# angeris/cfmm-routing-code

Hardware: NVIDIA H100
Metric: pools x dual-evaluations / second (1M constant-product pools, 4096 tokens); time to 1e-6 rel-gap reported beside it (higher is better)
Workload: dtype f64

## Files before the change

### cfmm_routing_code_b200/_lib.py

```python
from __future__ import annotations

import ctypes as C
import os

from . import build as _build

KIND_PRODUCT, KIND_SUM, KIND_GEOMEAN, KIND_BOUNDED = 0, 1, 2, 3

_ERRORS = {
    -1: "CFMM_E_NULL (required pointer is NULL)",
    -2: "CFMM_E_KIND (unknown kind / unsupported arity)",
    -3: "CFMM_E_SIZE (bad size)",
    -4: "CFMM_E_CUDA (CUDA runtime error)",
    -5: "CFMM_E_NODEVICE (no sm_90 device)",
    -6: "CFMM_E_STATE (handle used in the wrong state)",
}


class CfmmError(RuntimeError):
    pass


class Bucket(C.Structure):
    _fields_ = [
        ("kind", C.c_int32), ("arity", C.c_int32), ("n_pools", C.c_int64), ("stride", C.c_int64),
        ("reserves", C.c_void_p), ("tok_idx", C.c_void_p), ("gamma", C.c_void_p),
        ("weights", C.c_void_p), ("logrw", C.c_void_p), ("theta_bar", C.c_void_p),
    ]


class BlockedPairs(C.Structure):
    _fields_ = [
        ("n_pools", C.c_int64), ("n_tiles", C.c_int64), ("pools_per_tile", C.c_int32), ("reserved", C.c_int32),
        ("r0", C.c_void_p), ("r1", C.c_void_p), ("gamma_inv", C.c_void_p), ("lid", C.c_void_p),
        ("pos", C.c_void_p), ("rows", C.c_void_p), ("tok", C.c_void_p), ("desc", C.c_void_p),
    ]


class SolveParams(C.Structure):
    _fields_ = [("tol", C.c_double), ("nu_floor", C.c_double), ("max_iter", C.c_int32), ("cg_max", C.c_int32)]


class SolveResult(C.Structure):
    _fields_ = [("dual_value", C.c_double), ("primal_value", C.c_double), ("gap", C.c_double),
                ("primal_infeas", C.c_double), ("err", C.c_double), ("iters", C.c_int32), ("evals", C.c_int32),
                ("hvps", C.c_int32), ("status", C.c_int32)]


class PeerCtx(C.Structure):
    _fields_ = [("recv_acc_dev", C.c_void_p), ("recv_vec_dev", C.c_void_p), ("rank", C.c_int32), ("world", C.c_int32),
                ("seq_acc", C.c_uint64), ("seq_vec", C.c_uint64)]


class CsrPools(C.Structure):
    _fields_ = [("n_tokens", C.c_int32), ("n_pools", C.c_int64), ("nnz", C.c_int64), ("pool_ptr", C.c_void_p),
                ("tok_idx", C.c_void_p), ("reserves", C.c_void_p), ("weights", C.c_void_p), ("logrw", C.c_void_p),
                ("gamma", C.c_void_p), ("kind", C.c_void_p)]


class Batch(C.Structure):
    _fields_ = [("n_problems", C.c_int32), ("pool_range", C.c_void_p), ("c", C.c_void_p), ("a", C.c_void_p),
                ("flags", C.c_void_p), ("nu", C.c_void_p), ("psi", C.c_void_p), ("stats", C.c_void_p),
                ("delta", C.c_void_p), ("lambda_", C.c_void_p), ("trade_stride", C.c_int64)]


class BatchParams(C.Structure):
    _fields_ = [("tol", C.c_double), ("eps0", C.c_double), ("eps_min", C.c_double), ("eps_shrink", C.c_double),
                ("floor_rel", C.c_double), ("max_outer", C.c_int32), ("max_inner", C.c_int32)]


class EvalOut(C.Structure):
    _fields_ = [("delta", C.c_void_p), ("lambda_", C.c_void_p), ("hcoef", C.c_void_p), ("hmask", C.c_void_p)]


_lib = None


def lib_path() -> str:
    return _build.LIB


def load(build_if_missing: bool = True):
    global _lib
    if _lib is not None:
        return _lib
    path = _build.LIB
    if build_if_missing and _build.needs_build():
        try:
            _build.build_library()
        except Exception as e:
            if not os.path.exists(path):
                raise CfmmError(f"libcfmm_b200.so is missing and could not be built: {e}") from e
    if not os.path.exists(path):
        raise CfmmError("libcfmm_b200.so is missing: run `python -c 'import __graft_entry__ as g; g.build()'`")
    lib = C.CDLL(path)
    vp, i32, i64, dbl = C.c_void_p, C.c_int32, C.c_int64, C.c_double
    lib.cfmm_arb_eval.argtypes = [C.POINTER(Bucket), i32, vp, vp, dbl, vp, vp, C.POINTER(EvalOut), vp]
    lib.cfmm_arb_eval.restype = C.c_int
    for name in ("cfmm_hvp", "cfmm_hess_diag", "cfmm_hess_dense"):
        fn = getattr(lib, name)
        fn.restype = C.c_int
    lib.cfmm_hvp.argtypes = [C.POINTER(Bucket), i32, vp, vp, vp, vp, vp]
    lib.cfmm_hess_diag.argtypes = [C.POINTER(Bucket), i32, vp, vp, vp, vp]
    lib.cfmm_hess_dense.argtypes = [C.POINTER(Bucket), i32, vp, vp, vp, vp]
    lib.cfmm_blocked_layout_info.argtypes = [C.POINTER(i32)] * 4
    lib.cfmm_blocked_layout_info.restype = C.c_int
    lib.cfmm_set_blocked_config.argtypes = [i32]
    lib.cfmm_set_blocked_config.restype = C.c_int
    lib.cfmm_blocked_build_work_bytes.argtypes = [i64]
    lib.cfmm_blocked_build_work_bytes.restype = i64
    lib.cfmm_blocked_build.argtypes = [i64, i32, vp, vp, vp, C.POINTER(BlockedPairs), vp, vp, vp, i64, vp]
    lib.cfmm_blocked_build.restype = C.c_int
    lib.cfmm_blocked_eval.argtypes = [C.POINTER(BlockedPairs), i32, vp, vp, vp, C.POINTER(EvalOut), vp, i64, vp]
    lib.cfmm_blocked_eval.restype = C.c_int
    lib.cfmm_blocked_hvp.argtypes = [C.POINTER(BlockedPairs), i32, vp, vp, vp, vp, vp]
    lib.cfmm_blocked_hvp.restype = C.c_int
    lib.cfmm_blocked_diag.argtypes = [C.POINTER(BlockedPairs), i32, vp, vp, vp]
    lib.cfmm_blocked_diag.restype = C.c_int
    lib.cfmm_blocked_dense.argtypes = [C.POINTER(BlockedPairs), i32, vp, vp, vp]
    lib.cfmm_blocked_dense.restype = C.c_int
    lib.cfmm_blocked_solve_work_bytes.argtypes = [C.POINTER(BlockedPairs), i32]
    lib.cfmm_blocked_solve_work_bytes.restype = i64
    lib.cfmm_blocked_solve.argtypes = [C.POINTER(BlockedPairs), i32, vp, vp, vp, vp, vp, vp, vp,
                                       C.POINTER(SolveParams), C.POINTER(SolveResult), vp]
    lib.cfmm_blocked_solve.restype = C.c_int
    lib.cfmm_blocked_solve_peer.argtypes = [C.POINTER(BlockedPairs), i32, vp, vp, vp, vp, vp, vp, vp,
                                            C.POINTER(SolveParams), C.POINTER(SolveResult), C.POINTER(PeerCtx), vp]
    lib.cfmm_blocked_solve_peer.restype = C.c_int
    lib.cfmm_persist_solve_work_bytes.argtypes = [C.POINTER(BlockedPairs), i32]
    lib.cfmm_persist_solve_work_bytes.restype = i64
    lib.cfmm_persist_solve.argtypes = lib.cfmm_blocked_solve_peer.argtypes
    lib.cfmm_persist_solve.restype = C.c_int
    lib.cfmm_set_persist_cooperative.argtypes = [i32]
    lib.cfmm_set_persist_cooperative.restype = C.c_int
    lib.cfmm_persist_last_profile.argtypes = [vp]
    lib.cfmm_persist_last_profile.restype = C.c_int
    lib.cfmm_batch_solve_work_bytes.argtypes = [C.POINTER(CsrPools), i32, i64]
    lib.cfmm_batch_solve_work_bytes.restype = i64
    lib.cfmm_set_batch_lanes.argtypes = [i32]
    lib.cfmm_set_batch_lanes.restype = C.c_int
    lib.cfmm_batch_solve.argtypes = [C.POINTER(CsrPools), C.POINTER(Batch), C.POINTER(BatchParams), vp, vp]
    lib.cfmm_batch_solve.restype = C.c_int
    lib.cfmm_allreduce_ll.argtypes = [vp, vp, i32, i32, i32, i64, i64, vp, C.c_uint64, vp]
    lib.cfmm_allreduce_ll.restype = C.c_int
    lib.cfmm_sum_update_multipliers.argtypes = [C.POINTER(Bucket), vp, vp, vp, vp]
    lib.cfmm_sum_update_multipliers.restype = C.c_int
    lib.cfmm_zero.argtypes = [vp, i64, vp]
    lib.cfmm_zero.restype = C.c_int
    lib.cfmm_set_scatter_mode.argtypes = [i32]
    lib.cfmm_set_scatter_mode.restype = C.c_int
    lib.cfmm_launch_count.restype = i64
    lib.cfmm_reset_launch_count.restype = None
    lib.cfmm_last_cuda_error.restype = C.c_char_p
    lib.cfmm_version.restype = C.c_char_p
    if os.environ.get("CFMM_BATCH_LANES"):
        lib.cfmm_set_batch_lanes(int(os.environ["CFMM_BATCH_LANES"]))
    if os.environ.get("CFMM_BLOCKED_CFG"):
        for c in os.environ["CFMM_BLOCKED_CFG"].split(","):
            lib.cfmm_set_blocked_config(int(c))
    _lib = lib
    return lib


def check(rc: int, what: str = "cfmm call"):
    if rc != 0:
        extra = ""
        if rc == -4 and _lib is not None:
            extra = ": " + _lib.cfmm_last_cuda_error().decode()
        raise CfmmError(f"{what} failed: {_ERRORS.get(rc, rc)}{extra}")
```

### cfmm_routing_code_b200/csrc/cfmm_blocked.cu

```cuda
#include <math.h>

#include "cfmm_blocked.cuh"

using namespace cfmm;

namespace {

template <int P, int THREADS, int STAGES, int MODE , bool TRADES, bool HESS>
__global__ void __launch_bounds__(THREADS, kCtasPerSm)
k_blocked(const BlockedArgs A) {
    extern __shared__ __align__(128) unsigned char smem_raw[];
    __shared__ uint64_t full[STAGES];
    __shared__ double part[THREADS / 32];
    if (threadIdx.x == 0) {
        for (int s = 0; s < STAGES; ++s) mbar_init(&full[s], 1);
        mbar_fence_init();
    }
    __syncthreads();
    const long long t_beg = (A.n_tiles * (long long)blockIdx.x) / gridDim.x;
    const long long t_end = (A.n_tiles * (long long)(blockIdx.x + 1)) / gridDim.x;
    double acc = 0.0, acc2 = 0.0;
    unsigned phase = 0;
    blocked_pass<P, THREADS, STAGES, MODE, TRADES, HESS, false, true>(A, smem_raw, full, phase, t_beg, t_end, acc, acc2);
    if (MODE == 0) cta_accumulate<THREADS>(acc, part, A.arb);
}

template <int P>
struct __align__(128) TabStage {
    uint32_t rows[BlockedCfg<P>::kRowsMax];
    int32_t tok[BlockedCfg<P>::kTokMax];
    int4 desc;
};

template <int P>
__device__ __forceinline__ void issue_tables(TabStage<P>* st, uint64_t* bar, const BlockedArgs& A, long long tile,
                                             const int4 d) {
    const unsigned rows_b = round16(4u * (unsigned)d.y);
    const unsigned tok_b = round16(4u * (unsigned)d.x);
    mbar_expect_tx(bar, 16u + rows_b + tok_b);
    bulk_g2s(&st->desc, A.desc + tile, 16, bar);
    bulk_g2s(st->rows, A.rows + tile * BlockedCfg<P>::kRowsMax, rows_b, bar);
    bulk_g2s(st->tok, A.tok + tile * BlockedCfg<P>::kTokMax, tok_b, bar);
}

template <int NF>
struct PoolRegs {
    double a[NF];
    uint32_t lid, pos;
};

template <int P, int THREADS, int NF, int NPOOL>
__device__ __forceinline__ void load_pools(PoolRegs<NF> (&r)[NPOOL], const BlockedArgs& A, long long tile, int tid) {
    const long long toff = tile * P;
#pragma unroll
    for (int u = 0; u < NPOOL; ++u) {
        const long long q = toff + tid + u * THREADS;
#pragma unroll
        for (int k = 0; k < NF; ++k) r[u].a[k] = __ldg(A.slab[k] + q);
        r[u].lid = __ldg(A.lid + q);
        r[u].pos = __ldg(A.pos + q);
    }
}

template <int P, int NF>
__device__ __forceinline__ void prefetch_pools_l2(const BlockedArgs& A, long long tile) {
    constexpr int tp = P;
    const long long toff = tile * P;
#pragma unroll
    for (int k = 0; k < NF; ++k) bulk_prefetch_l2(A.slab[k] + toff, tp * 8);
    bulk_prefetch_l2(A.lid + toff, tp * 4);
    bulk_prefetch_l2(A.pos + toff, tp * 4);
}

template <int P, int THREADS, int STAGES, int MODE, bool TRADES, bool HESS>
__global__ void __launch_bounds__(THREADS, kCtasPerSm)
k_blocked_regs(const BlockedArgs A) {
    constexpr int NF = (MODE == 0) ? 3 : 1;
    constexpr int NPOOL = P / THREADS;
    constexpr int NPRE = (P + THREADS - 1) / THREADS;
    using St = TabStage<P>;
    extern __shared__ __align__(128) unsigned char smem_raw[];
    St* stages = reinterpret_cast<St*>(smem_raw);
    double* nul0 = reinterpret_cast<double*>(smem_raw + (size_t)STAGES * sizeof(St));
    double* g0 = nul0 + 2 * P;
    __shared__ uint64_t full[STAGES];
    __shared__ double part[THREADS / 32];
    const int tid = threadIdx.x, lane = tid & 31, warp = tid >> 5;
    const long long t_beg = (A.n_tiles * (long long)blockIdx.x) / gridDim.x;
    const long long t_end = (A.n_tiles * (long long)(blockIdx.x + 1)) / gridDim.x;
    if (tid == 0) {
        for (int s = 0; s < STAGES; ++s) mbar_init(&full[s], 1);
        mbar_fence_init();
    }
    __syncthreads();
    if (tid == 0) {
        for (int s = 0; s < STAGES; ++s) {
            const long long t = t_beg + s;
            if (t < t_end) issue_tables<P>(&stages[s], &full[s], A, t, __ldg(A.desc + t));
        }
        if (t_beg + 1 < t_end) prefetch_pools_l2<P, NF>(A, t_beg + 1);
        if (t_beg + 2 < t_end) prefetch_pools_l2<P, NF>(A, t_beg + 2);
    }
    PoolRegs<NF> cur[NPOOL], nxt[NPOOL];
    if (t_beg < t_end) load_pools<P, THREADS, NF, NPOOL>(cur, A, t_beg, tid);
    asm volatile("griddepcontrol.wait;" ::: "memory");
    asm volatile("griddepcontrol.launch_dependents;" ::: "memory");
    for (int j = blockIdx.x * THREADS + tid; j < A.n_zero; j += gridDim.x * THREADS) A.zero_next[j] = 0.0;
    double acc = 0.0;
    if (t_beg < t_end) {
        mbar_wait(&full[0], 0);
        if (MODE != 2) {
            const int ntok = stages[0].desc.x;
            for (int t = tid; t < ntok; t += THREADS) nul0[t] = __ldg(A.vec + stages[0].tok[t]);
        }
    }
    __syncthreads();
    int stage = 0, pstage = 0, buf = 0;
    unsigned parity = 0;
    for (long long tile = t_beg; tile < t_end; ++tile) {
        St& S = stages[stage];
        const double* nul = nul0 + buf * P;
        double* g = g0 + buf * 2 * P;
        const long long nx = tile + 1;
        int nstage = stage + 1;
        unsigned nparity = parity;
        if (nstage == STAGES) { nstage = 0; nparity ^= 1u; }
        double pre[NPRE];
        int ntok_n = 0;
        if (tid == 0 && tile + 3 < t_end) prefetch_pools_l2<P, NF>(A, tile + 3);
        if (nx < t_end) {
            load_pools<P, THREADS, NF, NPOOL>(nxt, A, nx, tid);
            mbar_wait(&full[nstage], nparity);
            if (MODE != 2) {
                ntok_n = stages[nstage].desc.x;
#pragma unroll
                for (int k = 0; k < NPRE; ++k) {
                    const int t = tid + k * THREADS;
                    pre[k] = (t < ntok_n) ? __ldg(A.vec + stages[nstage].tok[t]) : 0.0;
                }
            }
        }
        {
            double f0[NPOOL], f1[NPOOL];
#pragma unroll
            for (int u = 0; u < NPOOL; ++u) {
                const uint32_t li = cur[u].lid;
                if (MODE == 0) {
                    EvalOp::apply<TRADES, HESS>(A, tile * P + tid + u * THREADS, cur[u].a[0], cur[u].a[NF > 1 ? 1 : 0],
                                                cur[u].a[NF > 2 ? 2 : 0], nul[li & 0xffffu], nul[li >> 16], f0[u], f1[u],
                                                acc);
                } else if (MODE == 1) {
                    f0[u] = cur[u].a[0] * (nul[li & 0xffffu] - nul[li >> 16]);
                    f1[u] = -f0[u];
                } else {
                    f0[u] = cur[u].a[0];
                    f1[u] = f0[u];
                }
            }
#pragma unroll
            for (int u = 0; u < NPOOL; ++u) {
                g[cur[u].pos & 0xffffu] = f0[u];
                g[cur[u].pos >> 16] = f1[u];
            }
        }
        if (MODE != 2 && nx < t_end) {
            double* nn = nul0 + (buf ^ 1) * P;
#pragma unroll
            for (int k = 0; k < NPRE; ++k) {
                const int t = tid + k * THREADS;
                if (t < ntok_n) nn[t] = pre[k];
            }
        }
        __syncthreads();
        if (tid == 0 && tile > t_beg) {
            const long long far = tile - 1 + STAGES;
            if (far < t_end) {
                fence_proxy_async();
                issue_tables<P>(&stages[pstage], &full[pstage], A, far, __ldg(A.desc + far));
            }
        }
        const int nrow = S.desc.y;
        for (int r = tid; r < nrow; r += THREADS) {
            const uint32_t rw = S.rows[r];
            const double* q = g + row_start(rw);
            const int len = row_len(rw);
            double s0 = 0.0, s1 = 0.0;
            int k = 0;
#pragma unroll 1
            for (; k + 4 <= len; k += 4) { s0 += q[k] + q[k + 2]; s1 += q[k + 1] + q[k + 3]; }
            if (k + 2 <= len) { s0 += q[k]; s1 += q[k + 1]; k += 2; }
            if (k < len) s0 += q[k];
            const double s = s0 + s1;
            if (s != 0.0) atomicAdd(A.out + S.tok[row_tok(rw)], s);
        }
#pragma unroll
        for (int u = 0; u < NPOOL; ++u) cur[u] = nxt[u];
        pstage = stage; stage = nstage; parity = nparity; buf ^= 1;
    }
    if (MODE == 0) {
        acc = warp_sum(acc);
        if (lane == 0) part[warp] = acc;
        __syncthreads();
        if (tid < 32) {
            double s = (tid < THREADS / 32) ? part[tid] : 0.0;
            s = warp_sum(s);
            if (tid == 0 && s != 0.0) atomicAdd(A.arb, s);
        }
    }
}

__global__ void __launch_bounds__(256)
k_blocked_dense(long long n_pools, int n, const uint32_t* __restrict__ lid, const int32_t* __restrict__ tok,
                const double* __restrict__ hcoef, double* H) {
    for (long long q = (long long)blockIdx.x * blockDim.x + threadIdx.x; q < n_pools; q += (long long)gridDim.x * blockDim.x) {
        const double h = hcoef[q];
        if (h != 0.0) {
            const long long tile = q / kTileP;
            const uint32_t li = lid[q];
            const long long a = tok[tile * BlockedCfg<kTileP>::kTokMax + (li & 0xffffu)];
            const long long b = tok[tile * BlockedCfg<kTileP>::kTokMax + (li >> 16)];
            atomicAdd(H + a * n + a, h); atomicAdd(H + b * n + b, h);
            atomicAdd(H + a * n + b, -h); atomicAdd(H + b * n + a, -h);
        }
    }
}

int g_pdl = 1;
int g_row_cap = 32;

template <int MODE, bool TRADES, bool HESS>
int launch_tma(const BlockedArgs& A, cudaStream_t st) {
    constexpr int NF = (MODE == 0) ? 3 : 1;
    auto kern = k_blocked<kTileP, kTileT, kTileStages, MODE, TRADES, HESS>;
    const size_t sm = pass_smem_bytes<kTileP, kTileStages>(NF);
    static bool attr = false;
    if (!attr) {
        cudaFuncSetAttribute(kern, cudaFuncAttributeMaxDynamicSharedMemorySize, (int)sm);
        attr = true;
    }
    const long long cap = (long long)kCtasPerSm * num_sms();
    const int grid = (int)(A.n_tiles < cap ? A.n_tiles : cap);
    cudaLaunchConfig_t cfg = {};
    cfg.gridDim = dim3(grid); cfg.blockDim = dim3(kTileT); cfg.dynamicSmemBytes = sm; cfg.stream = st;
    cudaLaunchAttribute at[1];
    at[0].id = cudaLaunchAttributeProgrammaticStreamSerialization;
    at[0].val.programmaticStreamSerializationAllowed = g_pdl;
    cfg.attrs = at; cfg.numAttrs = 1;
    cudaLaunchKernelEx(&cfg, kern, A);
    return check_launch();
}

template <int MODE>
int launch_regs(const BlockedArgs& A, cudaStream_t st) {
    constexpr int P = kTileP, T = kTileT, S = 4;
    auto kern = k_blocked_regs<P, T, S, MODE, false, false>;
    const size_t sm = (size_t)S * sizeof(TabStage<P>) + (size_t)(2 * P + 4 * P) * sizeof(double);
    static bool attr = false;
    if (!attr) {
        cudaFuncSetAttribute(kern, cudaFuncAttributeMaxDynamicSharedMemorySize, (int)sm);
        attr = true;
    }
    const long long cap = (long long)kCtasPerSm * num_sms();
    const int grid = (int)(A.n_tiles < cap ? A.n_tiles : cap);
    cudaLaunchConfig_t cfg = {};
    cfg.gridDim = dim3(grid); cfg.blockDim = dim3(T); cfg.dynamicSmemBytes = sm; cfg.stream = st;
    cudaLaunchAttribute at[1];
    at[0].id = cudaLaunchAttributeProgrammaticStreamSerialization;
    at[0].val.programmaticStreamSerializationAllowed = g_pdl;
    cfg.attrs = at; cfg.numAttrs = 1;
    cudaLaunchKernelEx(&cfg, kern, A);
    return check_launch();
}

}

namespace cfmm {

int fill_blocked_args(const cfmm_blocked_pairs* b, BlockedArgs& A) {
    if (!b) return CFMM_E_NULL;
    if (b->pools_per_tile != kTileP) return CFMM_E_KIND;
    if (b->n_tiles < 0 || b->n_pools < 0 || b->n_pools > b->n_tiles * (int64_t)kTileP) return CFMM_E_SIZE;
    if (b->n_tiles > 0 && (!b->lid || !b->pos || !b->rows || !b->tok || !b->desc)) return CFMM_E_NULL;
    A.n_tiles = b->n_tiles;
    A.M = b->n_tiles * (int64_t)kTileP;
    A.lid = b->lid; A.pos = b->pos; A.rows = b->rows; A.tok = b->tok;
    A.desc = reinterpret_cast<const int4*>(b->desc);
    A.zero_next = nullptr; A.n_zero = 0;
    A.slab[0] = A.slab[1] = A.slab[2] = nullptr;
    A.vec = nullptr; A.vec2 = nullptr; A.beta = 0.0;
    A.out = nullptr; A.arb = nullptr; A.delta = A.lambda = A.hcoef = nullptr;
    return CFMM_OK;
}

}

extern "C" {

int cfmm_blocked_layout_info(int32_t* pools_per_tile, int32_t* rows_stride, int32_t* tok_stride, int32_t* row_cap) {
    if (pools_per_tile) *pools_per_tile = kTileP;
    if (rows_stride) *rows_stride = BlockedCfg<kTileP>::kRowsMax;
    if (tok_stride) *tok_stride = BlockedCfg<kTileP>::kTokMax;
    if (row_cap) *row_cap = g_row_cap;
    return CFMM_OK;
}

int cfmm_set_blocked_config(int32_t cfg) {
    if (cfg >= 300) { const int c = cfg - 300; if (c < 8 || c > 32) return CFMM_E_KIND; g_row_cap = c; return CFMM_OK; }
    if (cfg == 200 || cfg == 201) { g_pdl = cfg - 200; return CFMM_OK; }
    return CFMM_E_KIND;
}

int cfmm_blocked_eval(const cfmm_blocked_pairs* b, int32_t n_tokens, const double* nu, double* psi, double* arb,
                      const cfmm_eval_out* out, double* zero_next, int64_t n_zero, void* stream) {
    BlockedArgs A;
    int rc = fill_blocked_args(b, A);
    if (rc) return rc;
    if (n_tokens <= 0) return CFMM_E_SIZE;
    if (!nu || !psi || !arb) return CFMM_E_NULL;
    if (b->n_tiles == 0) return CFMM_OK;
    if (!b->r0 || !b->r1 || !b->gamma_inv) return CFMM_E_NULL;
    A.slab[0] = b->r0; A.slab[1] = b->r1; A.slab[2] = b->gamma_inv;
    A.vec = nu; A.out = psi; A.arb = arb;
    A.zero_next = zero_next; A.n_zero = zero_next ? (int)n_zero : 0;
    const bool trades = out && out->delta && out->lambda;
    const bool hess = out && out->hcoef;
    if (trades) { A.delta = out->delta; A.lambda = out->lambda; }
    if (hess) A.hcoef = out->hcoef;
    cudaStream_t st = static_cast<cudaStream_t>(stream);
    if (trades && hess) return launch_tma<0, true, true>(A, st);
    if (trades) return launch_tma<0, true, false>(A, st);
    if (hess) return launch_tma<0, false, true>(A, st);
    return launch_tma<0, false, false>(A, st);
}

int cfmm_blocked_hvp(const cfmm_blocked_pairs* b, int32_t n_tokens, const double* hcoef, const double* vt, double* y,
                     double* zero_next, void* stream) {
    BlockedArgs A;
    int rc = fill_blocked_args(b, A);
    if (rc) return rc;
    if (n_tokens <= 0) return CFMM_E_SIZE;
    if (!hcoef || !vt || !y) return CFMM_E_NULL;
    if (b->n_tiles == 0) return CFMM_OK;
    A.slab[0] = hcoef; A.vec = vt; A.out = y;
    A.zero_next = zero_next; A.n_zero = zero_next ? n_tokens : 0;
    return launch_regs<1>(A, static_cast<cudaStream_t>(stream));
}

int cfmm_blocked_dense(const cfmm_blocked_pairs* b, int32_t n_tokens, const double* hcoef, double* H, void* stream) {
    BlockedArgs A;
    int rc = fill_blocked_args(b, A);
    if (rc) return rc;
    if (n_tokens <= 0) return CFMM_E_SIZE;
    if (!hcoef || !H) return CFMM_E_NULL;
    if (b->n_tiles == 0) return CFMM_OK;
    const long long total = b->n_tiles * (long long)kTileP;
    const long long need = (total + 255) / 256, cap = 8LL * num_sms();
    k_blocked_dense<<<(int)(need < cap ? need : cap), 256, 0, static_cast<cudaStream_t>(stream)>>>(total, n_tokens, b->lid, b->tok, hcoef, H);
    return check_launch();
}

int cfmm_blocked_diag(const cfmm_blocked_pairs* b, int32_t n_tokens, const double* hcoef, double* diag, void* stream) {
    BlockedArgs A;
    int rc = fill_blocked_args(b, A);
    if (rc) return rc;
    if (n_tokens <= 0) return CFMM_E_SIZE;
    if (!hcoef || !diag) return CFMM_E_NULL;
    if (b->n_tiles == 0) return CFMM_OK;
    A.slab[0] = hcoef; A.out = diag;
    return launch_regs<2>(A, static_cast<cudaStream_t>(stream));
}

}
```

### cfmm_routing_code_b200/csrc/cfmm_blocked.cuh

```cuda
#pragma once
#include <math.h>

#include "cfmm_dev.cuh"

namespace cfmm {

#ifndef CFMM_TILE_P
#define CFMM_TILE_P 1024
#endif
#ifndef CFMM_CTAS_PER_SM
#define CFMM_CTAS_PER_SM 2
#endif
constexpr int kTileP = CFMM_TILE_P;
constexpr int kTileT = kTileP / 2;
constexpr int kTileStages = 2;
constexpr int kCtasPerSm = CFMM_CTAS_PER_SM;
static_assert(kTileP % 64 == 0 && kTileP <= 1024, "tile size: whole warps of two-pool threads, 10-bit local token ids");

template <int P>
struct BlockedCfg {
    static constexpr int kTokMax = P;
    static constexpr int kRowCapMin = 8;
    static constexpr int kRowsMax = P + 2 * P / kRowCapMin + 8;
};

template <int P, int NF>
struct __align__(128) Stage {
    double a[NF][P];
    uint32_t lid[P];
    uint32_t pos[P];
    uint32_t rows[BlockedCfg<P>::kRowsMax];
    int32_t tok[BlockedCfg<P>::kTokMax];
    int4 desc;
};

struct BlockedArgs {
    long long n_tiles;
    long long M;
    const double* slab[3];
    const uint32_t* lid;
    const uint32_t* pos;
    const uint32_t* rows;
    const int32_t* tok;
    const int4* desc;
    const double* vec;
    const double* vec2;
    double beta;
    double* out;
    double* zero_next;
    int n_zero;
    double* arb;
    double* delta;
    double* lambda;
    double* hcoef;
};

__device__ __forceinline__ unsigned round16(unsigned bytes) { return (bytes + 15u) & ~15u; }

template <int P, int NF>
__device__ __forceinline__ void issue_tile(Stage<P, NF>* st, uint64_t* bar, const BlockedArgs& A, long long tile,
                                           const int4 d) {
    const unsigned rows_b = round16(4u * (unsigned)d.y);
    const unsigned tok_b = round16(4u * (unsigned)d.x);
    const long long off = tile * P;
    mbar_expect_tx(bar, (unsigned)(NF * P * 8 + P * 4 + P * 4 + 16) + rows_b + tok_b);
    bulk_g2s(&st->desc, A.desc + tile, 16, bar);
#pragma unroll
    for (int k = 0; k < NF; ++k) bulk_g2s(st->a[k], A.slab[k] + off, P * 8, bar);
    bulk_g2s(st->lid, A.lid + off, P * 4, bar);
    bulk_g2s(st->pos, A.pos + off, P * 4, bar);
    bulk_g2s(st->rows, A.rows + tile * BlockedCfg<P>::kRowsMax, rows_b, bar);
    bulk_g2s(st->tok, A.tok + tile * BlockedCfg<P>::kTokMax, tok_b, bar);
}

__device__ __forceinline__ double clamp0(double x) {
    const int hi = __double2hiint(x);
    const int m = ~(hi >> 31);
    return __hiloint2double(hi & m, __double2loint(x) & m);
}

struct EvalOp {
    template <bool TRADES, bool HESS>
    __device__ __forceinline__ static void apply(const BlockedArgs& A, long long q, double R0, double R1, double gi,
                                                 double n0, double n1, double& f0, double& f1, double& acc) {
        const double p0 = n0 * R0, p1 = n1 * R1;
        const double w = p0 * p1 * gi;
        const double v = rsqrt(w);
        const double a = p0 * v, b = p1 * v;
        const double ob = 1.0 - b, oa = 1.0 - a;
        const double r0 = fma(-b, gi, 1.0), r1 = fma(-a, gi, 1.0);
        const double x0 = (ob < 0.0) ? ob * gi : clamp0(r0);
        const double x1 = (oa < 0.0) ? oa * gi : clamp0(r1);
        f0 = R0 * x0;
        f1 = R1 * x1;
        acc = fma(n0, f0, fma(n1, f1, acc));
        if (TRADES) {
            A.delta[q] = f0 < 0.0 ? -f0 : 0.0; A.delta[A.M + q] = f1 < 0.0 ? -f1 : 0.0;
            A.lambda[q] = f0 > 0.0 ? f0 : 0.0; A.lambda[A.M + q] = f1 > 0.0 ? f1 : 0.0;
        }
        if (HESS) A.hcoef[q] = (x0 != 0.0 || x1 != 0.0) ? 0.5 * w * v : 0.0;
    }
};

__device__ __forceinline__ int row_start(uint32_t r) { return (int)(r & 0xffffu); }
__device__ __forceinline__ int row_len(uint32_t r) { return (int)((r >> 16) & 0x3fu); }
__device__ __forceinline__ int row_tok(uint32_t r) { return (int)(r >> 22); }

template <bool COHERENT>
__device__ __forceinline__ double load_vec(const double* p) { return COHERENT ? *p : __ldg(p); }
template <int MODE, bool COHERENT>
__device__ __forceinline__ double gather_vec(const BlockedArgs& A, int t) {
    if (MODE == 1 && COHERENT) return fma(A.beta, A.vec[t], A.vec2[t]);
    return load_vec<COHERENT>(A.vec + t);
}

template <int P, int STAGES>
constexpr size_t pass_smem_bytes(int nf) {
    return (size_t)STAGES * (nf == 3 ? sizeof(Stage<P, 3>) : sizeof(Stage<P, 1>)) + (size_t)(3 * P) * sizeof(double);
}

template <int P, int THREADS, int STAGES, int MODE, bool TRADES, bool HESS, bool COHERENT, bool PDL>
__device__ __forceinline__ void blocked_pass(const BlockedArgs& A, unsigned char* smem_raw, uint64_t* full, unsigned& phase,
                                             long long t_beg, long long t_end, double& acc, double& acc2) {
    constexpr int NF = (MODE == 0) ? 3 : 1;
    using St = Stage<P, NF>;
    St* stages = reinterpret_cast<St*>(smem_raw);
    double* nul = reinterpret_cast<double*>(smem_raw + (size_t)STAGES * sizeof(St));
    double* g = nul + P;
    const int tid = threadIdx.x;
    if (tid == 0) {
        for (int s = 0; s < STAGES; ++s) {
            const long long t = t_beg + s;
            if (t < t_end) issue_tile<P, NF>(&stages[s], &full[s], A, t, __ldg(A.desc + t));
        }
    }
    if (PDL) {
        asm volatile("griddepcontrol.wait;" ::: "memory");
        asm volatile("griddepcontrol.launch_dependents;" ::: "memory");
    }
    for (int j = blockIdx.x * THREADS + tid; j < A.n_zero; j += gridDim.x * THREADS) A.zero_next[j] = 0.0;
    int stage = 0;
    constexpr int NPRE = (P + THREADS - 1) / THREADS;
    if (t_beg < t_end) {
        mbar_wait(&full[0], phase & 1u);
        if (MODE != 2) {
            const int ntok = stages[0].desc.x;
            for (int t = tid; t < ntok; t += THREADS) nul[t] = gather_vec<MODE, COHERENT>(A, stages[0].tok[t]);
        }
    }
    __syncthreads();
    for (long long tile = t_beg; tile < t_end; ++tile) {
        St& S = stages[stage];
        phase ^= 1u << stage;
        const int4 d = S.desc;
        const long long far = tile + STAGES;
        int4 dfar = make_int4(0, 0, 0, 0);
        if (tid == 0 && far < t_end) dfar = __ldg(A.desc + far);
        {
            constexpr int NPOOL = P / THREADS;
            double f0[NPOOL], f1[NPOOL];
            uint32_t ps[NPOOL];
#pragma unroll
            for (int u = 0; u < NPOOL; ++u) {
                const int l = tid + u * THREADS;
                const uint32_t li = S.lid[l];
                ps[u] = S.pos[l];
                if (MODE == 0) {
                    EvalOp::apply<TRADES, HESS>(A, tile * P + l, S.a[0][l], S.a[NF > 1 ? 1 : 0][l], S.a[NF > 2 ? 2 : 0][l],
                                                nul[li & 0xffffu], nul[li >> 16], f0[u], f1[u], acc);
                } else if (MODE == 1) {
                    const double pa = nul[li & 0xffffu], pb = nul[li >> 16], h = S.a[0][l];
                    f0[u] = h * (pa - pb);
                    f1[u] = -f0[u];
                    if (COHERENT) {
                        acc = fma(f0[u], pa - pb, acc);
                        acc2 = fma(h, fma(pa, pa, pb * pb), acc2);
                    }
                } else {
                    f0[u] = S.a[0][l];
                    f1[u] = f0[u];
                }
            }
#pragma unroll
            for (int u = 0; u < NPOOL; ++u) {
                g[ps[u] & 0xffffu] = f0[u];
                g[ps[u] >> 16] = f1[u];
            }
        }
        __syncthreads();
        const long long nxt = tile + 1;
        const int nstage = (stage + 1 == STAGES) ? 0 : stage + 1;
        double pre[NPRE];
        int ntok_n = 0;
        if (nxt < t_end) {
            mbar_wait(&full[nstage], (phase >> nstage) & 1u);
            if (MODE != 2) {
                ntok_n = stages[nstage].desc.x;
#pragma unroll
                for (int k = 0; k < NPRE; ++k) {
                    const int t = tid + k * THREADS;
                    pre[k] = (t < ntok_n) ? gather_vec<MODE, COHERENT>(A, stages[nstage].tok[t]) : 0.0;
                }
            }
        }
        for (int r = tid; r < d.y; r += THREADS) {
            const uint32_t rw = S.rows[r];
            const double* q = g + row_start(rw);
            const int len = row_len(rw);
            double s0 = 0.0, s1 = 0.0;
            int k = 0;
#pragma unroll 1
            for (; k + 4 <= len; k += 4) { s0 += q[k] + q[k + 2]; s1 += q[k + 1] + q[k + 3]; }
            if (k + 2 <= len) { s0 += q[k]; s1 += q[k + 1]; k += 2; }
            if (k < len) s0 += q[k];
            const double s = s0 + s1;
            if (s != 0.0) atomicAdd(A.out + S.tok[row_tok(rw)], s);
        }
        if (MODE != 2 && nxt < t_end) {
#pragma unroll
            for (int k = 0; k < NPRE; ++k) {
                const int t = tid + k * THREADS;
                if (t < ntok_n) nul[t] = pre[k];
            }
        }
        __syncthreads();
        if (tid == 0 && far < t_end) {
            fence_proxy_async();
            issue_tile<P, NF>(&S, &full[stage], A, far, dfar);
        }
        stage = nstage;
    }
}

template <int THREADS>
__device__ __forceinline__ void cta_accumulate(double acc, double* part, double* target) {
    const int tid = threadIdx.x;
    acc = warp_sum(acc);
    if ((tid & 31) == 0) part[tid >> 5] = acc;
    __syncthreads();
    if (tid < 32) {
        double s = (tid < THREADS / 32) ? part[tid] : 0.0;
        s = warp_sum(s);
        if (tid == 0 && s != 0.0) atomicAdd(target, s);
    }
}

int fill_blocked_args(const cfmm_blocked_pairs* b, BlockedArgs& A);

}
```

### cfmm_routing_code_b200/csrc/cfmm_layout.cu

```cuda
#include <cub/cub.cuh>

#include "cfmm_blocked.cuh"

using namespace cfmm;

namespace {

constexpr int LT = kTileT;
constexpr int LP = kTileP;
constexpr int LH = 2 * kTileP;
constexpr int LI = 4;
static_assert(LT * LI == LH, "block sort shape");
constexpr int LR = BlockedCfg<kTileP>::kRowsMax;

struct BuildArgs {
    long long m;
    int n_tokens, nb, row_cap, key_bits, tok_bits;
    const int32_t* idx;
    const double* R;
    const double* gamma;
    const uint32_t* order;
    double *r0, *r1, *gi;
    uint32_t *lid, *pos;
    uint32_t* rows;
    int32_t* tok;
    int4* desc;
    int32_t* status;
};

__global__ void __launch_bounds__(256)
k_pool_keys(long long m, int n_tokens, int nb, const int32_t* __restrict__ idx, const double* __restrict__ R,
            const double* __restrict__ gamma, uint32_t* __restrict__ keys, uint32_t* __restrict__ vals, int32_t* status) {
    int bad = 0;
    for (long long i = (long long)blockIdx.x * blockDim.x + threadIdx.x; i < m; i += (long long)gridDim.x * blockDim.x) {
        const int a = idx[2 * i], b = idx[2 * i + 1];
        const double R0 = R[2 * i], R1 = R[2 * i + 1], g = gamma[i];
        const bool ok = a >= 0 && a < n_tokens && b >= 0 && b < n_tokens && a != b && R0 > 0.0 && R1 > 0.0 && isfinite(R0) &&
                        isfinite(R1) && g > 0.0 && g <= 1.0;
        bad |= ok ? 0 : 1;
        const long long ba = ok ? ((long long)a * nb) / n_tokens : 0, bb = ok ? ((long long)b * nb) / n_tokens : 0;
        keys[i] = (uint32_t)((ba * nb + bb) * n_tokens + (ok ? a : 0));
        vals[i] = (uint32_t)i;
    }
    if (__syncthreads_or(bad) && threadIdx.x == 0) atomicAdd(status + 1, 1);
}

using Sort = cub::BlockRadixSort<uint32_t, LT, LI, uint32_t>;
using Scan = cub::BlockScan<int, LT>;

struct TileSmem {
    union { typename Sort::TempStorage sort; typename Scan::TempStorage scan; } tmp;
    uint32_t sk[LH];
    uint32_t sv[LH];
    uint16_t gid[LH];
    int gs[LP + 2];
    int rfirst[LP + 1];
    uint16_t rrank[LR + 8];
    int rstart[LR + 8];
    uint16_t lidh[LP][2], posh[LP][2];
    int ntok, nrow;
};

__global__ void __launch_bounds__(LT)
k_build_tiles(const BuildArgs B) {
    extern __shared__ __align__(16) unsigned char tile_smem_raw[];
    TileSmem& M = *reinterpret_cast<TileSmem*>(tile_smem_raw);
    auto& tmp = M.tmp;
    uint32_t* sk = M.sk; uint32_t* sv = M.sv; uint16_t* gid = M.gid; int* gs = M.gs; int* rfirst = M.rfirst;
    uint32_t* rk = M.sk;
    uint16_t* rrank = M.rrank; int* rstart = M.rstart;
    auto& lidh = M.lidh; auto& posh = M.posh;
    int& s_ntok = M.ntok; int& s_nrow = M.nrow;
    const int tid = threadIdx.x;
    const long long tile = blockIdx.x;
    const long long p0 = tile * LP;
    const int np = (int)(B.m - p0 < LP ? B.m - p0 : LP);
    const int nh = 2 * np;
    uint32_t key[LI], val[LI];
#pragma unroll
    for (int u = 0; u < LI; ++u) {
        const int h = tid * LI + u;
        const int slot = h >= LP ? 1 : 0, l = h - slot * LP;
        if (l < np) {
            const uint32_t pool = B.order[p0 + l];
            key[u] = (uint32_t)B.idx[2 * (long long)pool + slot];
            val[u] = (uint32_t)(slot << 15 | l);
        } else {
            key[u] = 0xffffffffu; val[u] = 0u;
        }
    }
    Sort(tmp.sort).Sort(key, val, 0, 32);
#pragma unroll
    for (int u = 0; u < LI; ++u) { sk[tid * LI + u] = key[u]; sv[tid * LI + u] = val[u]; }
    __syncthreads();
    int head[LI], gpre[LI];
#pragma unroll
    for (int u = 0; u < LI; ++u) {
        const int i = tid * LI + u;
        head[u] = (i < nh && (i == 0 || sk[i] != sk[i - 1])) ? 1 : 0;
    }
    int ntok;
    Scan(tmp.scan).ExclusiveSum(head, gpre, ntok);
    __syncthreads();
    const bool bad = ntok > LP;
#pragma unroll
    for (int u = 0; u < LI; ++u) {
        const int i = tid * LI + u;
        if (i < nh) {
            const int g = gpre[u] + head[u] - 1;
            gid[i] = (uint16_t)g;
            if (head[u] && !bad) { gs[g] = i; B.tok[tile * LP + g] = (int32_t)sk[i]; }
        }
    }
    if (tid == 0) { s_ntok = ntok; if (!bad) gs[ntok] = nh; }
    __syncthreads();
    if (bad) {
        if (tid == 0) { atomicAdd(B.status, 1); B.desc[tile] = make_int4(0, 0, 0, 0); }
        for (int l = tid; l < LP; l += LT) {
            B.r0[p0 + l] = 1.0; B.r1[p0 + l] = 1.0; B.gi[p0 + l] = 1.0; B.lid[p0 + l] = 0u; B.pos[p0 + l] = 0u;
        }
        return;
    }
    const int cap = B.row_cap;
    int nsub[2], rpre[2];
#pragma unroll
    for (int u = 0; u < 2; ++u) {
        const int g = tid * 2 + u;
        nsub[u] = g < ntok ? (gs[g + 1] - gs[g] + cap - 1) / cap : 0;
    }
    int nrow;
    Scan(tmp.scan).ExclusiveSum(nsub, rpre, nrow);
    __syncthreads();
#pragma unroll
    for (int u = 0; u < 2; ++u) {
        const int g = tid * 2 + u;
        if (g < ntok) {
            rfirst[g] = rpre[u];
            const int cnt = gs[g + 1] - gs[g];
            for (int s = 0; s < nsub[u]; ++s) {
                const int len = min(cap, cnt - cap * s);
                rk[rpre[u] + s] = (uint32_t)(63 - len) << 16 | (uint32_t)(rpre[u] + s);
            }
        }
    }
    if (tid == 0) s_nrow = nrow;
    __syncthreads();
    uint32_t rkey[LI], rdum[LI];
#pragma unroll
    for (int u = 0; u < LI; ++u) {
        const int r = tid * LI + u;
        rkey[u] = r < nrow ? rk[r] : 0xffffffffu;
        rdum[u] = 0u;
    }
    __syncthreads();
    Sort(tmp.sort).Sort(rkey, rdum, 0, 22);
    int rlen[LI], spre[LI];
#pragma unroll
    for (int u = 0; u < LI; ++u) {
        const int r = tid * LI + u;
        rlen[u] = r < nrow ? 63 - (int)(rkey[u] >> 16) : 0;
        if (r < nrow) rrank[rkey[u] & 0xffffu] = (uint16_t)r;
    }
    __syncthreads();
    int total;
    Scan(tmp.scan).ExclusiveSum(rlen, spre, total);
#pragma unroll
    for (int u = 0; u < LI; ++u) {
        const int r = tid * LI + u;
        if (r < nrow) { rstart[r] = spre[u]; rk[r] = (uint32_t)rlen[u]; }
    }
    __syncthreads();
    for (int i = tid; i < nh; i += LT) {
        const int g = gid[i], o = i - gs[g];
        const int r = rrank[rfirst[g] + o / cap];
        const int p = rstart[r] + o % cap;
        const uint32_t v = sv[i];
        const int slot = v >> 15, l = v & 0x7fffu;
        lidh[l][slot] = (uint16_t)g;
        posh[l][slot] = (uint16_t)p;
        if (o % cap == 0) B.rows[tile * LR + r] = (uint32_t)rstart[r] | rk[r] << 16 | (uint32_t)g << 22;
    }
    __syncthreads();
    for (int l = tid; l < LP; l += LT) {
        if (l < np) {
            const uint32_t pool = B.order[p0 + l];
            B.lid[p0 + l] = (uint32_t)lidh[l][0] | (uint32_t)lidh[l][1] << 16;
            B.pos[p0 + l] = (uint32_t)posh[l][0] | (uint32_t)posh[l][1] << 16;
            B.r0[p0 + l] = B.R[2 * (long long)pool]; B.r1[p0 + l] = B.R[2 * (long long)pool + 1];
            B.gi[p0 + l] = 1.0 / B.gamma[pool];
        } else {
            const int pl = l - np;
            B.lid[p0 + l] = 0u;
            B.pos[p0 + l] = (uint32_t)(nh + 2 * pl) | (uint32_t)(nh + 2 * pl + 1) << 16;
            B.r0[p0 + l] = 1.0; B.r1[p0 + l] = 1.0; B.gi[p0 + l] = 1.0;
        }
    }
    if (tid == 0) { B.desc[tile] = make_int4(s_ntok, s_nrow, 0, 0); atomicAdd(B.status + 2, s_nrow); }
}

inline size_t align_up(size_t x) { return (x + 255) & ~(size_t)255; }

size_t sort_temp_bytes(long long m) {
    size_t bytes = 0;
    cub::DeviceRadixSort::SortPairs(nullptr, bytes, (const uint32_t*)nullptr, (uint32_t*)nullptr, (const uint32_t*)nullptr,
                                    (uint32_t*)nullptr, (int)m, 0, 32);
    return bytes;
}

}

extern "C" {

int64_t cfmm_blocked_build_work_bytes(int64_t n_pools) {
    if (n_pools <= 0 || n_pools > 0x7fffffffLL) return CFMM_E_SIZE;
    return (int64_t)(4 * align_up(4 * (size_t)n_pools) + align_up(sort_temp_bytes(n_pools)));
}

int cfmm_blocked_build(int64_t n_pools, int32_t n_tokens, const int32_t* idx, const double* reserves, const double* gamma,
                       const cfmm_blocked_pairs* out, uint32_t* order, int32_t* status, void* work, int64_t work_bytes,
                       void* stream) {
    if (!idx || !reserves || !gamma || !out || !order || !status || !work) return CFMM_E_NULL;
    if (n_pools <= 0 || n_pools > 0x7fffffffLL || n_tokens <= 0) return CFMM_E_SIZE;
    if (work_bytes < cfmm_blocked_build_work_bytes(n_pools)) return CFMM_E_SIZE;
    const long long T = (n_pools + LP - 1) / LP;
    if (out->pools_per_tile != LP || out->n_tiles != T || out->n_pools != n_pools) return CFMM_E_SIZE;
    if (!out->r0 || !out->r1 || !out->gamma_inv || !out->lid || !out->pos || !out->rows || !out->tok || !out->desc) return CFMM_E_NULL;
    int row_cap = 32;
    cfmm_blocked_layout_info(nullptr, nullptr, nullptr, &row_cap);
    long long nb = (long long)llround(sqrt((double)n_pools / LP));
    if (nb < 1) nb = 1;
    if ((double)nb * nb * n_tokens >= 4294967296.0) return CFMM_E_SIZE;
    int key_bits = 1;
    while (key_bits < 32 && (1ull << key_bits) < (unsigned long long)(nb * nb) * (unsigned long long)n_tokens) ++key_bits;
    cudaStream_t st = static_cast<cudaStream_t>(stream);
    unsigned char* w = static_cast<unsigned char*>(work);
    auto take = [&](size_t bytes) { unsigned char* p = w; w += align_up(bytes); return p; };
    uint32_t* keys = reinterpret_cast<uint32_t*>(take(4 * (size_t)n_pools));
    uint32_t* vals = reinterpret_cast<uint32_t*>(take(4 * (size_t)n_pools));
    uint32_t* keys2 = reinterpret_cast<uint32_t*>(take(4 * (size_t)n_pools));
    take(4 * (size_t)n_pools);
    size_t temp_bytes = sort_temp_bytes(n_pools);
    void* temp = take(temp_bytes);
    cudaMemsetAsync(status, 0, 16, st);
    const int grid = (int)((n_pools + 255) / 256 < 4LL * num_sms() ? (n_pools + 255) / 256 : 4LL * num_sms());
    k_pool_keys<<<grid, 256, 0, st>>>(n_pools, n_tokens, (int)nb, idx, reserves, gamma, keys, vals, status);
    int rc = check_launch();
    if (rc) return rc;
    if (cub::DeviceRadixSort::SortPairs(temp, temp_bytes, keys, keys2, vals, order, (int)n_pools, 0, key_bits, st) != cudaSuccess) {
        g_last_err = cudaGetLastError();
        return CFMM_E_CUDA;
    }
    BuildArgs B;
    B.m = n_pools; B.n_tokens = n_tokens; B.nb = (int)nb; B.row_cap = row_cap; B.key_bits = key_bits; B.tok_bits = 32;
    B.idx = idx; B.R = reserves; B.gamma = gamma; B.order = order;
    B.r0 = const_cast<double*>(out->r0); B.r1 = const_cast<double*>(out->r1); B.gi = const_cast<double*>(out->gamma_inv);
    B.lid = const_cast<uint32_t*>(out->lid); B.pos = const_cast<uint32_t*>(out->pos);
    B.rows = const_cast<uint32_t*>(out->rows); B.tok = const_cast<int32_t*>(out->tok);
    B.desc = reinterpret_cast<int4*>(const_cast<int32_t*>(out->desc));
    B.status = status;
    static bool attr = false;
    if (!attr) {
        cudaFuncSetAttribute(k_build_tiles, cudaFuncAttributeMaxDynamicSharedMemorySize, (int)sizeof(TileSmem));
        attr = true;
    }
    k_build_tiles<<<(int)T, LT, sizeof(TileSmem), st>>>(B);
    return check_launch();
}

}
```

### cfmm_routing_code_b200/csrc/cfmm_persist.cu

```cuda
#include <math.h>
#include <string.h>

#include "cfmm_blocked.cuh"

using namespace cfmm;

namespace {

constexpr int PT = kTileT;
constexpr unsigned long long kSpinLimit = 6000000000ull;


struct DevResult {
    double dual_value, primal_value, gap, primal_infeas, err;
    int iters, evals, hvps, status;
    unsigned long long seq_acc, seq_vec;
    long long prof[16];
};

struct PersistArgs {
    BlockedArgs B;
    int n;
    const double *c, *a;
    const unsigned char *eq, *fixed;
    double* nu[2];
    double* acc[2];
    double *y, *diag, *hcoef;
    double *lb, *grad[2], *fr[2], *pg[2], *dt, *x, *r, *z, *p, *minv;
    unsigned* ctl;
    double tol, nu_floor;
    int max_iter, cg_max;
    LLCell* const* recv_acc;
    LLCell* const* recv_vec;
    int rank, world;
    unsigned long long seq_acc, seq_vec;
    double* nu_out;
    double* psi_out;
    DevResult* res;
};

__device__ __forceinline__ unsigned ld_acquire_gpu(const unsigned* p) {
    unsigned v;
    asm volatile("ld.acquire.gpu.global.u32 %0, [%1];" : "=r"(v) : "l"(p) : "memory");
    return v;
}

struct Kkt { double err, g, primal, infeas, lin; };

template <int MODE>
__device__ __forceinline__ void run_pass(const PersistArgs& S, const double* vec, double* out, unsigned char* smem_raw,
                                         uint64_t* full, unsigned& phase, long long t_beg, long long t_end, double* part,
                                         double beta) {
    BlockedArgs A = S.B;
    A.vec = vec; A.out = out; A.zero_next = nullptr; A.n_zero = 0;
    asm volatile("fence.proxy.async;" ::: "memory");
    if (MODE == 0) { A.arb = out + S.n; A.hcoef = S.hcoef; }
    else A.slab[0] = S.hcoef;
    if (MODE == 1) { A.vec2 = S.z; A.beta = beta; }
    double acc = 0.0, acc2 = 0.0;
    blocked_pass<kTileP, PT, kTileStages, MODE, false, MODE == 0, true, false>(A, smem_raw, full, phase, t_beg, t_end, acc, acc2);
    if (MODE == 0) {
        cta_accumulate<PT>(acc, part, A.arb);
        asm volatile("fence.proxy.async;" ::: "memory");
    }
    if (MODE == 1) {
        cta_accumulate<PT>(acc, part, out + S.n);
        __syncthreads();
        cta_accumulate<PT>(acc2, part, out + S.n + 1);
    }
}

__device__ __forceinline__ double ldw(const double* p) { return *p; }

constexpr int kSliceMax = 256;
constexpr int kQ = 10;

enum { PH_KKT = 1, PH_DIAG = 2, PH_HVP = 3, PH_STEP = 4, PH_DONE = 5 };

struct DistArgs {
    PersistArgs P;
    double* accr[2];
    double* y2[2];
    double* partial;
    int nsl;
};

struct DState {
    int phase, set, cur, iters, evals, hvps, status, cg_k, ls, yb, first_step, dir_ok, aborted, parity;
    double err, g0, rz, r0n, eta, alpha, lin1, beta, al, imx, thr;
    int flat;
    Kkt kc;
    unsigned long long seq_acc, seq_vec;
    unsigned bar;
    long long prof[16];
};

__device__ __forceinline__ void grid_barrier(unsigned* ctl, DState* ds) {
    __threadfence();
    __syncthreads();
    if (threadIdx.x == 0) {
        const unsigned target = (++ds->bar) * gridDim.x;
        atomicAdd(ctl, 1u);
        const long long t0 = clock64();
        while (ld_acquire_gpu(ctl) < target) {
            if (ld_acquire_gpu(ctl + 32) != 0u) { ds->aborted = 1; break; }
            if ((unsigned long long)(clock64() - t0) > kSpinLimit) { ctl[32] = 1u; ds->aborted = 1; break; }
        }
    }
    __syncthreads();
}

__device__ __forceinline__ void ll_push(double mine, LLCell* const* recv, long long slot, long long stride, int j, int rank,
                                        int world, unsigned long long seq) {
    for (int r = 0; r < world; ++r)
        if (r != rank) st_ll(recv[r] + slot + (long long)rank * stride + j, mine, seq);
}
__device__ __noinline__ double ll_poll_sum(double mine, LLCell* const* recv, long long slot, long long stride, int j,
                                           int rank, int world, unsigned long long seq, unsigned* ctl) {
    const LLCell* base = recv[rank] + slot + j;
    const long long t0 = clock64();
    double s = 0.0;
    for (int r0 = 0; r0 < world; r0 += 4) {
        double v0 = 0.0, v1 = 0.0, v2 = 0.0, v3 = 0.0;
        unsigned pending = 0u;
#pragma unroll
        for (int k = 0; k < 4; ++k)
            if (r0 + k < world && r0 + k != rank) pending |= 1u << k;
        unsigned spins = 0u;
        while (pending) {
            double t[4];
            unsigned long long f[4];
#pragma unroll
            for (int k = 0; k < 4; ++k)
                if (pending >> k & 1u) ld_ll(base + (long long)(r0 + k) * stride, t[k], f[k]);
            if ((pending & 1u) && f[0] == seq) { v0 = t[0]; pending &= ~1u; }
            if ((pending & 2u) && f[1] == seq) { v1 = t[1]; pending &= ~2u; }
            if ((pending & 4u) && f[2] == seq) { v2 = t[2]; pending &= ~4u; }
            if ((pending & 8u) && f[3] == seq) { v3 = t[3]; pending &= ~8u; }
            if (pending && (++spins & 63u) == 0u && (unsigned long long)(clock64() - t0) > kSpinLimit) { ctl[32] = 1u; break; }
        }
        if (r0 + 0 < world) s += (r0 + 0 == rank) ? mine : v0;
        if (r0 + 1 < world) s += (r0 + 1 == rank) ? mine : v1;
        if (r0 + 2 < world) s += (r0 + 2 == rank) ? mine : v2;
        if (r0 + 3 < world) s += (r0 + 3 == rank) ? mine : v3;
    }
    return s;
}

template <bool MULTI>
__global__ void __launch_bounds__(PT, kCtasPerSm)
k_solve_dist(const __grid_constant__ DistArgs D) {
    extern __shared__ __align__(128) unsigned char smem_raw[];
    __shared__ uint64_t full[kTileStages];
    __shared__ double part[PT / 32];
    __shared__ double tot[kQ];
    __shared__ DState ds;
    const PersistArgs& S = D.P;
    const int tid = threadIdx.x, lane = tid & 31, warp = tid >> 5;
    const int n = S.n, nsl = D.nsl, G = gridDim.x;
    if (tid == 0) {
        for (int s = 0; s < kTileStages; ++s) mbar_init(&full[s], 1);
        mbar_fence_init();
        ds.phase = PH_KKT; ds.set = 0; ds.cur = 0; ds.iters = 0; ds.evals = 0; ds.hvps = 0; ds.status = 1; ds.cg_k = 0; ds.ls = 0;
        ds.yb = 0; ds.first_step = 1; ds.dir_ok = 0; ds.aborted = 0; ds.parity = 0; ds.flat = 0;
        ds.err = INFINITY; ds.g0 = 0.0; ds.rz = 0.0; ds.r0n = 0.0; ds.eta = 0.1; ds.alpha = 1.0; ds.lin1 = 0.0; ds.beta = 0.0;
        ds.al = 0.0; ds.imx = 0.0; ds.thr = 1e-5;
        ds.kc.err = INFINITY; ds.kc.g = 0.0; ds.kc.primal = 0.0; ds.kc.infeas = 0.0; ds.kc.lin = 0.0;
        ds.seq_acc = S.seq_acc; ds.seq_vec = S.seq_vec; ds.bar = 0;
        for (int k = 0; k < 16; ++k) ds.prof[k] = 0;
    }
    __syncthreads();
    const long long t_beg = (S.B.n_tiles * (long long)blockIdx.x) / G;
    const long long t_end = (S.B.n_tiles * (long long)(blockIdx.x + 1)) / G;
    unsigned phase_bits = 0;
    for (int s0 = blockIdx.x + warp * G; s0 < nsl; s0 += (PT / 32) * G) {
        const int lo = (int)((long long)n * s0 / nsl), hi = (int)((long long)n * (s0 + 1) / nsl);
        for (int j = lo + lane; j < hi; j += 32) {
            const double l = S.eq[j] ? S.nu_floor : fmax(S.c[j], S.nu_floor);
            S.lb[j] = l;
            S.nu[0][j] = S.fixed[j] ? S.c[j] : fmax(S.nu[0][j], l);
            S.acc[0][j] = 0.0;
        }
        if (s0 == nsl - 1 && lane == 0) S.acc[0][n] = 0.0;
    }
    grid_barrier(S.ctl, &ds);
    for (;;) {
        const int phase = ds.phase, set = ds.set, cur = ds.cur;
        if (phase == PH_DONE || ds.aborted) break;
        const long long tp0 = clock64();
        if (phase == PH_KKT) run_pass<0>(S, S.nu[set], S.acc[set], smem_raw, full, phase_bits, t_beg, t_end, part, 0.0);
        else if (phase == PH_HVP) run_pass<1>(S, S.p, D.y2[ds.yb], smem_raw, full, phase_bits, t_beg, t_end, part, ds.beta);
        else if (phase == PH_DIAG) run_pass<2>(S, nullptr, S.diag, smem_raw, full, phase_bits, t_beg, t_end, part, 0.0);
        const long long tp1 = clock64();
        if (phase != PH_STEP) grid_barrier(S.ctl, &ds);
        const long long tp2 = clock64();
        const int par = ds.parity;
        double* P0 = D.partial + (size_t)par * kQ * kSliceMax;
        constexpr bool multi = MULTI;
        unsigned long long seq = 0;
        if (phase == PH_KKT) seq = ds.seq_acc + 1; else if (phase == PH_DIAG || phase == PH_HVP) seq = ds.seq_vec + 1;
        const long long slot_acc = (long long)(seq % 3) * S.world * (n + 1), slot_vec = (long long)(seq % 3) * S.world * (n + 2);
        if (phase == PH_HVP) {
            const double* yb = D.y2[ds.yb];
            if (multi) {
                for (int s0 = blockIdx.x + warp * G; s0 < nsl; s0 += (PT / 32) * G) {
                    const int lo = (int)((long long)n * s0 / nsl), hi = (int)((long long)n * (s0 + 1) / nsl);
                    for (int j = lo + lane; j < hi; j += 32) ll_push(ldw(yb + j), S.recv_vec, slot_vec, n + 2, j, S.rank, S.world, seq);
                    if (s0 == nsl - 1 && lane < 2) ll_push(ldw(yb + n + lane), S.recv_vec, slot_vec, n + 2, n + lane, S.rank, S.world, seq);
                }
            }
            if (tid == 0) {
                double pHp = ldw(yb + n), pdp = ldw(yb + n + 1);
                if (multi) {
                    pHp = ll_poll_sum(pHp, S.recv_vec, slot_vec, n + 2, n, S.rank, S.world, seq, S.ctl);
                    pdp = ll_poll_sum(pdp, S.recv_vec, slot_vec, n + 2, n + 1, S.rank, S.world, seq, S.ctl);
                }
                ds.flat = pHp <= 1e-14 * pdp;
                ds.al = ds.flat ? 0.0 : ds.rz / pHp;
            }
            __syncthreads();
        }
        const double al = ds.al;
        const int flat = ds.flat;
        for (int s0 = blockIdx.x + warp * G; s0 < nsl; s0 += (PT / 32) * G) {
            const int lo = (int)((long long)n * s0 / nsl), hi = (int)((long long)n * (s0 + 1) / nsl);
            double q[kQ];
#pragma unroll
            for (int k = 0; k < kQ; ++k) q[k] = 0.0;
            for (int j = lo + lane; j < hi; j += 32) {
                if (phase == PH_KKT) {
                    double pj = ldw(S.acc[set] + j);
                    const double nj = ldw(S.nu[set] + j), aj = S.a[j], cj = S.c[j], lbj = ldw(S.lb + j);
                    const unsigned char ej = S.eq[j], fj = S.fixed[j];
                    const bool wl = set != cur;
                    const double np = wl ? ldw(S.nu[cur] + j) : 0.0, gp = wl ? ldw(S.grad[cur] + j) : 0.0;
                    if (multi) {
                        ll_push(pj, S.recv_acc, slot_acc, n + 1, j, S.rank, S.world, seq);
                        if (s0 == nsl - 1 && lane == 0) ll_push(ldw(S.acc[set] + n), S.recv_acc, slot_acc, n + 1, n, S.rank, S.world, seq);
                        pj = ll_poll_sum(pj, S.recv_acc, slot_acc, n + 1, j, S.rank, S.world, seq, S.ctl);
                    }
                    const double g = aj + pj;
                    const bool near = (nj <= lbj * (1.0 + ds.thr)) && !ej;
                    const bool act = fj || (near && g > 0.0);
                    const double f = act ? 0.0 : 1.0, v = nj * g * f;
                    S.grad[set][j] = g; S.fr[set][j] = f; S.pg[set][j] = v; D.accr[set][j] = pj;
                    S.diag[j] = 0.0;
                    q[0] += fabs(v); q[1] += (nj - cj) * aj; q[2] += nj * fabs(g); q[3] += cj * pj;
                    q[4] += nj * (fj ? 0.0 : (ej ? fabs(g) : fmax(-g, 0.0)));
                    q[5] += gp * (nj - np);
                    q[6] = fmax(q[6], fabs(g) * f);
                    q[7] = fmax(q[7], fmax(fabs(aj), fj ? 0.0 : fabs(pj)));
                } else if (phase == PH_DIAG) {
                    double d = ldw(S.diag + j);
                    const double f = ldw(S.fr[cur] + j), g = ldw(S.pg[cur] + j);
                    if (multi) {
                        ll_push(d, S.recv_vec, slot_vec, n + 2, j, S.rank, S.world, seq);
                        d = ll_poll_sum(d, S.recv_vec, slot_vec, n + 2, j, S.rank, S.world, seq, S.ctl);
                    }
                    const double mi = f / fmax(d, 1e-300), r = -g, z = mi * r;
                    S.minv[j] = mi; S.x[j] = 0.0; S.r[j] = r; S.z[j] = z; S.p[j] = z;
                    D.y2[0][j] = 0.0;
                    q[0] += r * z;
                    q[6] = fmax(q[6], fabs(g));
                } else if (phase == PH_HVP) {
                    double yv = ldw(D.y2[ds.yb] + j);
                    const double pp = ldw(S.p + j), zz = ldw(S.z + j), xx = ldw(S.x + j), rr = ldw(S.r + j),
                                 mm = ldw(S.minv + j), g = ldw(S.pg[cur] + j);
                    if (multi) yv = ll_poll_sum(yv, S.recv_vec, slot_vec, n + 2, j, S.rank, S.world, seq, S.ctl);
                    const double pj = fma(ds.beta, pp, zz);
                    double xn = xx;
                    S.p[j] = pj;
                    if (flat) {
                        if (ds.cg_k == 0) { xn = pj; S.x[j] = xn; }
                    } else {
                        const double r = rr - al * yv, z = mm * r;
                        xn = fma(al, pj, xx);
                        S.x[j] = xn; S.r[j] = r; S.z[j] = z;
                        q[0] += r * z;
                    }
                    q[1] += g * xn;
                    D.y2[ds.yb ^ 1][j] = 0.0;
                } else {
                    const double g = ldw(S.pg[cur] + j), xx = ldw(S.x + j), v = ldw(S.nu[cur] + j), l = ldw(S.lb + j);
                    double d;
                    if (ds.first_step) { d = ds.dir_ok ? xx : -g * ds.imx; S.dt[j] = d; }
                    else d = ldw(S.dt + j);
                    const double e = fmin(fmax(ds.alpha * d, -20.0), 20.0);
                    S.nu[cur ^ 1][j] = S.fixed[j] ? S.c[j] : fmax(v * exp(e), l);
                    S.acc[cur ^ 1][j] = 0.0;
                }
            }
            if (s0 == nsl - 1 && lane == 0) {
                if (phase == PH_KKT) {
                    double arb = ldw(S.acc[set] + n);
                    if (multi) arb = ll_poll_sum(arb, S.recv_acc, slot_acc, n + 1, n, S.rank, S.world, seq, S.ctl);
                    q[8] = arb;
                } else if (phase == PH_DIAG) { D.y2[0][n] = 0.0; D.y2[0][n + 1] = 0.0; }
                else if (phase == PH_HVP) { D.y2[ds.yb ^ 1][n] = 0.0; D.y2[ds.yb ^ 1][n + 1] = 0.0; }
                else S.acc[cur ^ 1][n] = 0.0;
            }
            if (phase != PH_STEP) {
#pragma unroll
                for (int k = 0; k < 6; ++k) q[k] = warp_sum(q[k]);
                q[6] = warp_max(q[6]); q[7] = warp_max(q[7]);
                if (lane == 0) {
#pragma unroll
                    for (int k = 0; k < 9; ++k) P0[k * kSliceMax + s0] = q[k];
                }
            }
        }
        const long long tp3 = clock64();
        grid_barrier(S.ctl, &ds);
        const long long tp4 = clock64();
        if (warp < 9 && phase != PH_STEP) {
            const int k = warp;
            const bool is_max = k == 6 || k == 7;
            double t = 0.0;
            for (int s = lane; s < nsl; s += 32) {
                const double v = ldw(P0 + k * kSliceMax + s);
                t = is_max ? fmax(t, v) : t + v;
            }
            t = is_max ? warp_max(t) : warp_sum(t);
            if (lane == 0) tot[k] = t;
        }
        __syncthreads();
        if (tid == 0) {
            ds.parity ^= 1;
            int next = PH_DONE;
            bool newton = false;
            if (ds.aborted) {
                next = PH_DONE;
            } else if (phase == PH_KKT) {
                ++ds.seq_acc; ++ds.evals;
                Kkt k;
                k.g = tot[1] + tot[8];
                k.err = fmax(tot[0] / fmax(fmax(fabs(k.g), 1e-3 * tot[2]), 1e-300), tot[6] / fmax(tot[7], 1e-300));
                k.primal = tot[3]; k.infeas = tot[4] / fmax(fabs(k.g), 1e-300); k.lin = tot[5];
                if (set == cur) {
                    ds.kc = k; ds.err = k.err; ds.g0 = k.g; newton = true;
                } else {
                    if (ds.ls == 0) ds.lin1 = k.lin;
                    bool accept = k.g <= ds.g0 + 1e-4 * k.lin, stalled = false;
                    if (!accept && (fabs(k.g - ds.g0) <= 1e-13 * fabs(ds.g0) || fabs(ds.lin1) <= 1e-9 * fabs(ds.g0))) {
                        if (k.err < 0.99 * ds.err) accept = true;
                        else if (ds.alpha < 1e-3) stalled = true;
                    }
                    if (accept) { ds.cur = set; ds.kc = k; ds.err = k.err; ds.g0 = k.g; newton = true; }
                    else if (stalled || ++ds.ls >= 50) { ds.status = 2; next = PH_DONE; }
                    else { ds.alpha *= 0.5; ds.first_step = 0; next = PH_STEP; }
                }
                if (newton) {
                    if (ds.iters >= S.max_iter) { ds.status = 1; next = PH_DONE; }
                    else {
                        ++ds.iters;
                        if (ds.err <= S.tol) { ds.status = 0; next = PH_DONE; }
                        else next = PH_DIAG;
                    }
                }
            } else if (phase == PH_DIAG) {
                ++ds.seq_vec;
                ds.rz = tot[0]; ds.r0n = sqrt(fmax(ds.rz, 0.0)); ds.eta = fmin(0.1, sqrt(ds.err));
                ds.imx = 1.0 / fmax(tot[6], 1e-300);
                ds.cg_k = 0; ds.beta = 0.0; ds.yb = 0;
                if (ds.rz <= 0.0) { ds.dir_ok = 0; ds.first_step = 1; ds.alpha = 1.0; ds.ls = 0; ds.lin1 = 0.0; next = PH_STEP; }
                else next = PH_HVP;
            } else if (phase == PH_HVP) {
                ++ds.seq_vec; ++ds.hvps;
                bool stop = flat != 0;
                if (!flat) {
                    const double rzn = tot[0];
                    stop = (rzn <= 0.0) || (sqrt(fmax(rzn, 0.0)) <= ds.eta * ds.r0n);
                    ds.beta = rzn / ds.rz;
                    ds.rz = rzn;
                }
                ++ds.cg_k; ds.yb ^= 1;
                if (!stop && ds.cg_k < S.cg_max) next = PH_HVP;
                else {
                    const double sdir = tot[1];
                    ds.dir_ok = (isfinite(sdir) && sdir < 0.0) ? 1 : 0;
                    ds.first_step = 1; ds.alpha = 1.0; ds.ls = 0; ds.lin1 = 0.0;
                    next = PH_STEP;
                }
            } else {
                ds.set = cur ^ 1;
                ds.thr = fmin(1e-2, fmax(1e-3 * (isfinite(ds.err) ? ds.err : 1e-2), 1e-14));
                next = PH_KKT;
            }
            if (next == PH_DONE && ds.status == 1 && ds.err <= S.tol) ds.status = 0;
            ds.phase = next;
            if (blockIdx.x == 0) {
                ds.prof[phase == PH_KKT ? 0 : phase == PH_HVP ? 1 : phase == PH_DIAG ? 2 : 7] += tp1 - tp0;
                ds.prof[3] += tp2 - tp1; ds.prof[4] += tp3 - tp2; ds.prof[5] += tp4 - tp3; ds.prof[6] += clock64() - tp4;
            }
        }
        __syncthreads();
    }
    {
        const int cur = ds.cur;
        for (int s0 = blockIdx.x + warp * G; s0 < nsl; s0 += (PT / 32) * G) {
            const int lo = (int)((long long)n * s0 / nsl), hi = (int)((long long)n * (s0 + 1) / nsl);
            for (int j = lo + lane; j < hi; j += 32) {
                S.psi_out[j] = ldw(D.accr[cur] + j);
                if (cur != 0) S.nu_out[j] = ldw(S.nu[cur] + j);
            }
        }
        if (blockIdx.x == 0 && tid == 0) {
            DevResult R;
            R.dual_value = ds.kc.g; R.primal_value = ds.kc.primal;
            R.gap = (ds.kc.g - ds.kc.primal) / fmax(fabs(ds.kc.g), 1e-300);
            R.primal_infeas = ds.kc.infeas; R.err = ds.err;
            R.iters = ds.iters; R.evals = ds.evals; R.hvps = ds.hvps; R.status = ds.aborted ? 3 : ds.status;
            R.seq_acc = ds.seq_acc; R.seq_vec = ds.seq_vec;
            for (int k = 0; k < 16; ++k) R.prof[k] = ds.prof[k];
            *S.res = R;
        }
    }
}

inline size_t align_up(size_t x) { return (x + 255) & ~(size_t)255; }
thread_local long long g_last_prof[16] = {0};
int g_persist_cooperative = 1;

}

extern "C" {

int64_t cfmm_persist_solve_work_bytes(const cfmm_blocked_pairs* b, int32_t n_tokens) {
    if (!b || n_tokens <= 0) return CFMM_E_SIZE;
    const size_t n = (size_t)n_tokens;
    size_t bytes = align_up(8 * (size_t)b->n_tiles * (size_t)b->pools_per_tile);
    bytes += 2 * align_up(8 * (n + 1));
    bytes += 18 * align_up(8 * n) + align_up(8 * (n + 2));
    bytes += align_up(512) + align_up(sizeof(DevResult));
    bytes += 2 * align_up(8 * n) + 2 * align_up(8 * (n + 2)) + align_up(8 * (size_t)2 * kQ * kSliceMax);
    return (int64_t)bytes;
}

int cfmm_persist_solve(const cfmm_blocked_pairs* b, int32_t n_tokens, const double* c, const double* a,
                       const uint8_t* eq, const uint8_t* pinned, double* nu, double* psi_out, void* work,
                       const cfmm_solve_params* prm, cfmm_solve_result* res, cfmm_peer_ctx* peer, void* stream) {
    if (!b || !c || !a || !eq || !pinned || !nu || !psi_out || !work || !prm || !res) return CFMM_E_NULL;
    if (n_tokens <= 0 || b->n_tiles <= 0) return CFMM_E_SIZE;
    if (!b->r0 || !b->r1 || !b->gamma_inv) return CFMM_E_NULL;
    if (peer && (!peer->recv_acc_dev || !peer->recv_vec_dev)) return CFMM_E_NULL;
    if (peer && (peer->world < 2 || peer->world > 16 || peer->rank < 0 || peer->rank >= peer->world)) return CFMM_E_SIZE;
    cudaStream_t st = static_cast<cudaStream_t>(stream);
    PersistArgs S;
    memset(&S, 0, sizeof(S));
    int rc = fill_blocked_args(b, S.B);
    if (rc) return rc;
    S.B.slab[0] = b->r0; S.B.slab[1] = b->r1; S.B.slab[2] = b->gamma_inv;
    const int n = n_tokens;
    S.n = n; S.c = c; S.a = a; S.eq = eq; S.fixed = pinned;
    unsigned char* w = static_cast<unsigned char*>(work);
    auto take = [&](size_t bytes) { unsigned char* p = w; w += align_up(bytes); return p; };
    auto vec = [&]() { return reinterpret_cast<double*>(take(8 * (size_t)n)); };
    S.hcoef = reinterpret_cast<double*>(take(8 * (size_t)S.B.M));
    S.acc[0] = reinterpret_cast<double*>(take(8 * (size_t)(n + 1)));
    S.acc[1] = reinterpret_cast<double*>(take(8 * (size_t)(n + 1)));
    S.nu[0] = nu; S.nu[1] = vec();
    S.y = reinterpret_cast<double*>(take(8 * (size_t)(n + 2))); S.diag = vec(); S.lb = vec();
    S.grad[0] = vec(); S.grad[1] = vec(); S.fr[0] = vec(); S.fr[1] = vec(); S.pg[0] = vec(); S.pg[1] = vec();
    S.dt = vec(); S.x = vec(); S.r = vec(); S.z = vec(); S.p = vec(); S.minv = vec();
    vec(); vec(); vec();
    S.ctl = reinterpret_cast<unsigned*>(take(512));
    S.res = reinterpret_cast<DevResult*>(take(sizeof(DevResult)));
    S.tol = prm->tol; S.nu_floor = prm->nu_floor; S.max_iter = prm->max_iter; S.cg_max = prm->cg_max;
    S.nu_out = nu; S.psi_out = psi_out;
    if (peer) {
        S.recv_acc = static_cast<LLCell* const*>(const_cast<void*>(peer->recv_acc_dev));
        S.recv_vec = static_cast<LLCell* const*>(const_cast<void*>(peer->recv_vec_dev));
        S.rank = peer->rank; S.world = peer->world; S.seq_acc = peer->seq_acc; S.seq_vec = peer->seq_vec;
    } else {
        S.rank = 0; S.world = 1;
    }
    DistArgs D;
    D.accr[0] = vec(); D.accr[1] = vec();
    D.y2[0] = reinterpret_cast<double*>(take(8 * (size_t)(n + 2))); D.y2[1] = reinterpret_cast<double*>(take(8 * (size_t)(n + 2)));
    D.partial = reinterpret_cast<double*>(take(8 * (size_t)2 * kQ * kSliceMax));
    D.nsl = (n + 15) / 16 < kSliceMax ? ((n + 15) / 16 > 0 ? (n + 15) / 16 : 1) : kSliceMax;
    D.P = S;
    const size_t sm = pass_smem_bytes<kTileP, kTileStages>(3);
    const bool multi = S.world > 1;
    auto kern = multi ? k_solve_dist<true> : k_solve_dist<false>;
    static int occs[2] = {-1, -1};
    int& occ = occs[multi ? 1 : 0];
    if (occ < 0) {
        int o = -1;
        cudaError_t e = cudaFuncSetAttribute(kern, cudaFuncAttributeMaxDynamicSharedMemorySize, (int)sm);
        if (e == cudaSuccess) e = cudaOccupancyMaxActiveBlocksPerMultiprocessor(&o, kern, PT, sm);
        if (e != cudaSuccess || o < 1) { g_last_err = e; return CFMM_E_CUDA; }
        occ = o;
    }
    const long long cap = (long long)occ * num_sms();
    const int grid = (int)(S.B.n_tiles < cap ? S.B.n_tiles : cap);
    cudaMemsetAsync(S.ctl, 0, 512, st);
    cudaLaunchConfig_t cfg = {};
    cfg.gridDim = dim3(grid); cfg.blockDim = dim3(PT); cfg.dynamicSmemBytes = sm; cfg.stream = st;
    cudaLaunchAttribute at[1];
    at[0].id = cudaLaunchAttributeCooperative;
    at[0].val.cooperative = g_persist_cooperative;
    cfg.attrs = at; cfg.numAttrs = 1;
    cudaLaunchKernelEx(&cfg, kern, D);
    rc = check_launch();
    if (rc) return rc;
    static thread_local DevResult* hres = nullptr;
    if (!hres && cudaHostAlloc(&hres, sizeof(DevResult), cudaHostAllocDefault) != cudaSuccess) return CFMM_E_CUDA;
    cudaMemcpyAsync(hres, S.res, sizeof(DevResult), cudaMemcpyDeviceToHost, st);
    if (cudaStreamSynchronize(st) != cudaSuccess) { g_last_err = cudaGetLastError(); return CFMM_E_CUDA; }
    res->dual_value = hres->dual_value; res->primal_value = hres->primal_value; res->gap = hres->gap;
    res->primal_infeas = hres->primal_infeas; res->err = hres->err;
    res->iters = hres->iters; res->evals = hres->evals; res->hvps = hres->hvps; res->status = hres->status;
    if (peer) { peer->seq_acc = hres->seq_acc; peer->seq_vec = hres->seq_vec; }
    for (int k = 0; k < 16; ++k) g_last_prof[k] = hres->prof[k];
    return hres->status == 3 ? CFMM_E_STATE : CFMM_OK;
}

int cfmm_set_persist_cooperative(int32_t on) {
    if (on != 0 && on != 1) return CFMM_E_KIND;
    g_persist_cooperative = on;
    return CFMM_OK;
}

int cfmm_persist_last_profile(int64_t* out8) {
    if (!out8) return CFMM_E_NULL;
    for (int k = 0; k < 16; ++k) out8[k] = g_last_prof[k];
    return CFMM_OK;
}

}
```

### cfmm_routing_code_b200/pools.py

```python
from __future__ import annotations

import ctypes as C
import dataclasses
from typing import Dict, List, Optional, Sequence

import numpy as np
import torch

from . import _lib

KIND_GEOMEAN_HOST = 0
KIND_SUM_HOST = 1
KIND_BOUNDED_HOST = 3


@dataclasses.dataclass
class HostPools:
    n_tokens: int
    pool_ptr: np.ndarray
    tok_idx: np.ndarray
    reserves: np.ndarray
    weights: np.ndarray
    gamma: np.ndarray
    kind: np.ndarray

    @property
    def m(self) -> int:
        return int(len(self.gamma))

    @staticmethod
    def from_lists(n_tokens, local_indices, reserves, fees, kinds, weights=None) -> "HostPools":
        m = len(local_indices)
        if not (len(reserves) == len(fees) == len(kinds) == m):
            raise ValueError("local_indices, reserves, fees, kinds must have one entry per pool")
        ptr = [0]; idx: List[int] = []; res: List[float] = []; wts: List[float] = []; kd: List[int] = []
        for i, l in enumerate(local_indices):
            k = len(l)
            if len(reserves[i]) != k:
                raise ValueError(f"pool {i}: {len(reserves[i])} reserves for {k} tokens")
            if len(set(int(t) for t in l)) != k:
                raise ValueError(f"pool {i}: repeated token in local_indices")
            ptr.append(ptr[-1] + k)
            idx += [int(t) for t in l]
            res += [float(x) for x in reserves[i]]
            if kinds[i] == "sum":
                if k != 2:
                    raise ValueError("constant-sum pools must have 2 tokens (as arbitrage.py:11)")
                kd.append(KIND_SUM_HOST); wts += [0.0] * k
            elif kinds[i] == "bounded_product":
                o = None if (weights is None or weights[i] is None) else np.asarray(weights[i], float)
                if k != 2 or o is None or len(o) != 2 or np.any(o < 0) or not np.all(np.isfinite(o)):
                    raise ValueError(f"pool {i}: bounded_product needs 2 tokens and 2 non-negative offsets in weights[i]")
                kd.append(KIND_BOUNDED_HOST); wts += list(o)
            elif kinds[i] in ("geomean", "product"):
                w = np.ones(k) if (weights is None or weights[i] is None) else np.asarray(weights[i], float)
                if len(w) != k or np.any(w <= 0):
                    raise ValueError(f"pool {i}: bad weights")
                kd.append(KIND_GEOMEAN_HOST); wts += list(w / w.sum())
            else:
                raise ValueError(f"pool {i}: unknown kind {kinds[i]!r}")
        return HostPools(int(n_tokens), np.asarray(ptr, np.int64), np.asarray(idx, np.int32),
                         np.asarray(res, np.float64), np.asarray(wts, np.float64),
                         np.asarray(fees, np.float64), np.asarray(kd, np.uint8))

    @staticmethod
    def from_pairs(n_tokens, idx, reserves, gamma) -> "HostPools":
        m = len(gamma)
        hp = HostPools(int(n_tokens), np.arange(0, 2 * m + 1, 2, dtype=np.int64),
                       np.ascontiguousarray(idx, np.int32).reshape(-1),
                       np.ascontiguousarray(reserves, np.float64).reshape(-1),
                       np.full(2 * m, 0.5), np.ascontiguousarray(gamma, np.float64), np.zeros(m, np.uint8))
        hp._uniform_product = True
        return hp

    def pin_memory(self) -> "HostPools":
        keep = []
        for name in ("tok_idx", "reserves", "weights", "gamma", "kind", "pool_ptr"):
            t = torch.from_numpy(np.ascontiguousarray(getattr(self, name))).pin_memory()
            keep.append(t)
            setattr(self, name, t.numpy())
        self._pinned = keep
        return self

    def validate(self):
        slot_kind = np.repeat(np.asarray(self.kind), np.diff(self.pool_ptr)) if np.any(self.kind == KIND_BOUNDED_HOST) else None
        virt = self.reserves if slot_kind is None else self.reserves + np.where(slot_kind == KIND_BOUNDED_HOST, self.weights, 0.0)
        lo_ok = np.all(self.reserves > 0) if slot_kind is None else np.all(self.reserves >= 0) and np.all(virt > 0)
        if not lo_ok or not np.all(np.isfinite(self.reserves)):
            raise ValueError("reserves must be positive and finite (bounded_product: >= 0 with positive virtual reserves)")
        if np.any(self.gamma <= 0) or np.any(self.gamma > 1):
            raise ValueError("fees (gamma) must lie in (0, 1]")
        if self.tok_idx.min(initial=0) < 0 or self.tok_idx.max(initial=0) >= self.n_tokens:
            raise ValueError("token index out of range")


class BucketSpec:

    def __init__(self, hp: HostPools, kind: int, arity: int, sel: Optional[np.ndarray], lo: int = 0,
                 hi: Optional[int] = None):
        self.hp, self.kind, self.arity, self._sel = hp, kind, arity, sel
        self.lo, self.hi = int(lo), int(hp.m if hi is None else hi)
        self._contiguous = sel is None
        self.m = (self.hi - self.lo) if sel is None else int(len(sel))
        self._off = None

    @property
    def identity(self) -> bool:
        return self._contiguous

    @property
    def sel(self) -> np.ndarray:
        if self._sel is None:
            self._sel = np.arange(self.lo, self.hi, dtype=np.int64)
        return self._sel

    @property
    def off(self) -> np.ndarray:
        if self._off is None:
            self._off = self.hp.pool_ptr[self.sel][None, :] + np.arange(self.arity)[:, None]
        return self._off

    def subset(self, local_idx: np.ndarray) -> "BucketSpec":
        return BucketSpec(self.hp, self.kind, self.arity, self.sel[local_idx])


def split_buckets(hp: HostPools, rank: int = 0, world: int = 1) -> List["BucketSpec"]:
    m = hp.m
    if m == 0:
        return []
    if getattr(hp, "_uniform_product", False):
        lo, hi = (m * rank) // world, (m * (rank + 1)) // world
        return [BucketSpec(hp, _lib.KIND_PRODUCT, 2, None, lo, hi)]
    uniform_pairs = int(hp.pool_ptr[-1]) == 2 * m and (hp.pool_ptr[1] - hp.pool_ptr[0]) == 2 and \
        bool(np.all(np.diff(hp.pool_ptr[::max(1, m // 64)]) == 2 * max(1, m // 64))) and \
        bool(np.array_equal(hp.pool_ptr[:3], np.arange(0, 2 * min(m, 2) + 1, 2)[:3]))
    if uniform_pairs:
        uniform_pairs = bool(np.all(np.diff(hp.pool_ptr) == 2))
    if uniform_pairs and not hp.kind.any() and bool(np.all(hp.weights == 0.5)):
        lo, hi = (m * rank) // world, (m * (rank + 1)) // world
        return [BucketSpec(hp, _lib.KIND_PRODUCT, 2, None, lo, hi)]
    ar = np.diff(hp.pool_ptr)
    first = hp.pool_ptr[:-1]
    is_cp = (hp.kind == KIND_GEOMEAN_HOST) & (ar == 2)
    is_cp &= (hp.weights[first] == 0.5) & (hp.weights[np.minimum(first + 1, len(hp.weights) - 1)] == 0.5)
    keys = []
    if is_cp.any():
        keys.append((_lib.KIND_PRODUCT, 2, np.nonzero(is_cp)[0]))
    cs = hp.kind == KIND_SUM_HOST
    if cs.any():
        if np.any(ar[cs] != 2):
            raise ValueError("constant-sum pools must have 2 tokens")
        keys.append((_lib.KIND_SUM, 2, np.nonzero(cs)[0]))
    bp = hp.kind == KIND_BOUNDED_HOST
    if bp.any():
        if np.any(ar[bp] != 2):
            raise ValueError("bounded_product pools must have 2 tokens")
        keys.append((_lib.KIND_BOUNDED, 2, np.nonzero(bp)[0]))
    gm = (hp.kind == KIND_GEOMEAN_HOST) & ~is_cp
    for k in np.unique(ar[gm]).tolist():
        if k < 2 or k > 32:
            raise ValueError(f"weighted pools support 2..32 tokens, got {k}")
        keys.append((_lib.KIND_GEOMEAN, int(k), np.nonzero(gm & (ar == k))[0]))
    out = []
    for kind, k, sel in keys:
        if world > 1:
            lo = (len(sel) * rank) // world
            hi = (len(sel) * (rank + 1)) // world
            sel = sel[lo:hi]
        out.append(BucketSpec(hp, kind, k, sel))
    return out


TILE = 1024


def _padded(arr2d: np.ndarray, stride: int, fill) -> np.ndarray:
    k, m = arr2d.shape
    out = np.full((k, stride), fill, dtype=arr2d.dtype)
    out[:, :m] = arr2d
    return out


class DeviceBucket:
    def __init__(self, hp: HostPools, spec, device):
        self.kind = spec.kind; self.arity = spec.arity
        self.spec = spec
        self.m = spec.m
        self.stride = max(TILE, -(-self.m // TILE) * TILE)
        f64 = dict(dtype=torch.float64, device=device)
        self.weights = self.logrw = self.theta_bar = None
        if spec.identity and self.arity == 2 and int(hp.pool_ptr[-1]) == 2 * hp.m:
            m, lo, hi = self.m, spec.lo, spec.hi
            self.reserves = torch.ones((2, self.stride), **f64)
            self.reserves[:, :m] = torch.from_numpy(hp.reserves[2 * lo:2 * hi]).to(device).view(m, 2).t()
            self.tok_idx = torch.zeros((2, self.stride), dtype=torch.int32, device=device)
            self.tok_idx[:, :m] = torch.from_numpy(hp.tok_idx[2 * lo:2 * hi]).to(device).view(m, 2).t()
            self.gamma = torch.ones(self.stride, **f64)
            self.gamma[:m] = torch.from_numpy(hp.gamma[lo:hi]).to(device)
            R = W = None
        else:
            R = hp.reserves[spec.off]
            self.reserves = torch.as_tensor(_padded(R, self.stride, 1.0), **f64)
            self.tok_idx = torch.as_tensor(_padded(hp.tok_idx[spec.off].astype(np.int32), self.stride, 0),
                                           dtype=torch.int32, device=device)
            self.gamma = torch.as_tensor(_padded(hp.gamma[spec.sel][None, :], self.stride, 1.0)[0], **f64)
        if self.kind == _lib.KIND_GEOMEAN:
            W = hp.weights[spec.off]
            self.weights = torch.as_tensor(_padded(W, self.stride, 1.0), **f64)
            self.logrw = torch.as_tensor(_padded(np.log(R / W), self.stride, 0.0), **f64)
        if self.kind == _lib.KIND_BOUNDED:
            self.weights = torch.as_tensor(_padded(hp.weights[spec.off], self.stride, 1.0), **f64)
        if self.kind == _lib.KIND_SUM:
            self.theta_bar = torch.zeros((2, self.stride), **f64)
        self.delta = self.lam = self.hcoef = self.hmask = None
        self._device = device
        self.c_bucket = _lib.Bucket(
            self.kind, self.arity, self.m, self.stride, self.reserves.data_ptr(), self.tok_idx.data_ptr(),
            self.gamma.data_ptr(),
            self.weights.data_ptr() if self.weights is not None else None,
            self.logrw.data_ptr() if self.logrw is not None else None,
            self.theta_bar.data_ptr() if self.theta_bar is not None else None)

    @property
    def sel(self) -> np.ndarray:
        return self.spec.sel

    @property
    def off(self) -> np.ndarray:
        return self.spec.off

    def bytes_resident(self) -> int:
        n = 0
        for t in (self.reserves, self.tok_idx, self.gamma, self.weights, self.logrw, self.theta_bar):
            if t is not None:
                n += t.numel() * t.element_size()
        return n

    def out_struct(self, trades: bool, hess: bool):
        f64 = dict(dtype=torch.float64, device=self._device)
        if trades and self.delta is None:
            self.delta = torch.zeros((self.arity, self.stride), **f64)
            self.lam = torch.zeros((self.arity, self.stride), **f64)
        if hess and self.hcoef is None:
            self.hcoef = torch.zeros(self.stride, **f64)
            self.hmask = torch.zeros(self.stride, dtype=torch.int32, device=self._device)
        return _lib.EvalOut(self.delta.data_ptr() if trades else None, self.lam.data_ptr() if trades else None,
                            self.hcoef.data_ptr() if hess else None, self.hmask.data_ptr() if hess else None)


def blocked_layout_info(lib):
    v = [C.c_int32() for _ in range(4)]
    _lib.check(lib.cfmm_blocked_layout_info(*[C.byref(x) for x in v]), "cfmm_blocked_layout_info")
    return tuple(int(x.value) for x in v)


def build_blocked_pairs(idx: torch.Tensor, n_tokens: int, P: int, rows_stride: int, tok_stride: int, row_cap: int):
    dev = idx.device
    m = idx.shape[1]
    i64 = dict(dtype=torch.int64, device=dev)
    nb = max(1, int(round((m / P) ** 0.5)))
    a, b = idx[0], idx[1]
    key = ((a * nb // n_tokens) * nb + (b * nb // n_tokens)) * n_tokens + a
    order = torch.argsort(key, stable=True)
    residual = []
    for _pass in range(4):
        mm = order.numel()
        if mm == 0:
            break
        pos = torch.arange(mm, **i64)
        ntiles = -(-mm // P)
        tile = pos // P
        he_tok = torch.cat([a[order], b[order]])
        he_tile = torch.cat([tile, tile])
        ck, perm = torch.sort(he_tile * n_tokens + he_tok, stable=True)
        uniq, inv, counts = torch.unique_consecutive(ck, return_inverse=True, return_counts=True)
        u_tile = uniq // n_tokens
        ntok = torch.bincount(u_tile, minlength=ntiles)
        bad = ntok > tok_stride
        if not bool(bad.any()):
            break
        if _pass == 3:
            residual.append(order); order = order[:0]; mm = 0
            break
        keep = ~bad[tile]
        residual.append(order[~keep])
        order = order[keep]
    residual = torch.cat(residual) if residual else order[:0]
    if order.numel() == 0:
        return order, residual, None
    U = uniq.numel()
    tok_off = torch.cumsum(ntok, 0) - ntok
    ltok_u = torch.arange(U, **i64) - tok_off[u_tile]
    he_ltok = torch.empty(2 * mm, **i64)
    he_ltok[perm] = ltok_u[inv]
    M = ntiles * P
    lid = torch.zeros(M, dtype=torch.int32, device=dev)
    lid[:mm] = (he_ltok[:mm] | (he_ltok[mm:] << 16)).to(torch.int32)
    tok = torch.zeros((ntiles, tok_stride), dtype=torch.int32, device=dev)
    tok[u_tile, ltok_u] = (uniq - u_tile * n_tokens).to(torch.int32)
    nsub = (counts + row_cap - 1) // row_cap
    n_rows = int(nsub.sum())
    first_row_u = torch.cumsum(nsub, 0) - nsub
    row_u = torch.repeat_interleave(torch.arange(U, **i64), nsub)
    sub = torch.arange(n_rows, **i64) - first_row_u[row_u]
    g_start = torch.cumsum(counts, 0) - counts
    row_tile0 = u_tile[row_u]
    row_len0 = torch.clamp(counts[row_u] - row_cap * sub, max=row_cap)
    srt = torch.argsort(row_tile0 * 64 + (63 - row_len0), stable=True)
    rank = torch.empty_like(srt); rank[srt] = torch.arange(n_rows, **i64)
    row_tile, row_len, row_ltok = row_tile0[srt], row_len0[srt], ltok_u[row_u][srt]
    nrow = torch.bincount(row_tile, minlength=ntiles)
    row_first = torch.cumsum(nrow, 0) - nrow
    r_local = torch.arange(n_rows, **i64) - row_first[row_tile]
    if int(nrow.max()) > rows_stride:
        raise _lib.CfmmError("blocked layout: row table overflow (library/builder mismatch)")
    cs = torch.cumsum(row_len, 0) - row_len
    row_start = cs - cs[row_first][row_tile]
    he_o = torch.arange(2 * mm, **i64) - g_start[inv]
    he_row = rank[first_row_u[inv] + he_o // row_cap]
    he_pos = torch.empty(2 * mm, **i64)
    he_pos[perm] = row_start[he_row] + he_o % row_cap
    pos = torch.zeros(M, dtype=torch.int32, device=dev)
    pad_base = 2 * (mm - (ntiles - 1) * P)
    if M > mm:
        padl = torch.arange(M - mm, **i64)
        pos[mm:] = ((pad_base + 2 * padl) | ((pad_base + 2 * padl + 1) << 16)).to(torch.int32)
    pos[:mm] = (he_pos[:mm] | (he_pos[mm:] << 16)).to(torch.int32)
    rows = torch.zeros((ntiles, rows_stride), dtype=torch.int32, device=dev)
    word = row_start | (row_len << 16) | (row_ltok << 22)
    rows[row_tile, r_local] = torch.where(word >= 2 ** 31, word - 2 ** 32, word).to(torch.int32)
    desc = torch.stack([ntok, nrow, torch.zeros_like(ntok), torch.zeros_like(ntok)], 1).to(torch.int32).contiguous()
    tables = dict(n_tiles=ntiles, M=M, lid=lid, tok=tok, pos=pos, rows=rows, desc=desc,
                  rows_per_pool=n_rows / mm, tok_per_tile=float(ntok.double().mean()))
    return order, residual, tables


class BlockedBucket:
    kind = _lib.KIND_PRODUCT
    arity = 2
    blocked = True

    def __init__(self, hp: HostPools, spec, device, lib):
        self.spec = spec
        P, rows_stride, tok_stride, row_cap = blocked_layout_info(lib)
        f64 = dict(dtype=torch.float64, device=device)
        self.theta_bar = None
        self.delta = self.lam = self.hcoef = self.hmask = None
        self._device = device
        self._sel = self._off = None
        if spec.identity and int(hp.pool_ptr[-1]) == 2 * hp.m and self._build_native(hp, spec, device, lib, P, rows_stride, tok_stride):
            return
        if spec.identity:
            lo, hi = spec.lo, spec.hi
            R = torch.from_numpy(hp.reserves[2 * lo:2 * hi]).to(device, non_blocking=True).view(-1, 2)
            idx = torch.from_numpy(hp.tok_idx[2 * lo:2 * hi]).to(device, non_blocking=True).view(-1, 2).to(torch.int64)
            gam = torch.from_numpy(hp.gamma[lo:hi]).to(device, non_blocking=True)
            if getattr(hp, "_validate_on_device", False):
                chk = torch.stack([R.min(), gam.min(), 1.0 - gam.max(), idx.min().double(),
                                   float(hp.n_tokens - 1) - idx.max().double(),
                                   torch.isfinite(R).all().double() - 0.5]).cpu()
                if bool((chk[:2] <= 0).any()) or bool((chk[2:] < 0).any()):
                    raise ValueError("invalid pool data (reserves > 0, fees in (0, 1], token ids in range, finite)")
        else:
            R = torch.as_tensor(np.ascontiguousarray(hp.reserves[spec.off].T), **f64)
            idx = torch.as_tensor(np.ascontiguousarray(hp.tok_idx[spec.off].T).astype(np.int64), device=device)
            gam = torch.as_tensor(np.ascontiguousarray(hp.gamma[spec.sel]), **f64)
        order, residual, t = build_blocked_pairs(idx.t(), hp.n_tokens, P, rows_stride, tok_stride, row_cap)
        self.order = order
        self.residual = residual.cpu().numpy() if residual.numel() else np.zeros(0, np.int64)
        self.m = int(order.numel())
        if self.m == 0:
            self.tables = None
            return
        self.tables = t
        self.stride = t["M"]

        def slab(vals, fill):
            out = torch.full((t["M"],), fill, **f64)
            out[:self.m] = vals
            return out
        self.r0 = slab(R[order, 0], 1.0)
        self.r1 = slab(R[order, 1], 1.0)
        self.gamma_inv = slab(1.0 / gam[order], 1.0)
        self.c_blocked = _lib.BlockedPairs(self.m, t["n_tiles"], P, 0, self.r0.data_ptr(), self.r1.data_ptr(),
                                           self.gamma_inv.data_ptr(), t["lid"].data_ptr(), t["pos"].data_ptr(),
                                           t["rows"].data_ptr(), t["tok"].data_ptr(), t["desc"].data_ptr())

    def _build_native(self, hp, spec, device, lib, P, rows_stride, tok_stride) -> bool:
        lo, hi = spec.lo, spec.hi
        m = hi - lo
        if m <= 0:
            return False
        nb = max(1, int(round((m / P) ** 0.5)))
        if nb * nb * hp.n_tokens >= 2 ** 32 or m >= 2 ** 31:
            return False
        T = -(-m // P)
        M = T * P
        f64 = dict(dtype=torch.float64, device=device)
        i32 = dict(dtype=torch.int32, device=device)
        idx = torch.from_numpy(np.ascontiguousarray(hp.tok_idx[2 * lo:2 * hi], np.int32)).to(device, non_blocking=True)
        R = torch.from_numpy(hp.reserves[2 * lo:2 * hi]).to(device, non_blocking=True)
        gam = torch.from_numpy(hp.gamma[lo:hi]).to(device, non_blocking=True)
        slabs = torch.empty((3, M), **f64)
        words = torch.empty((2, M), **i32)
        rows = torch.empty((T, rows_stride), **i32)
        tok = torch.empty((T, tok_stride), **i32)
        desc = torch.empty((T, 4), **i32)
        order = torch.empty(m, **i32)
        status = torch.empty(4, **i32)
        nbytes = int(lib.cfmm_blocked_build_work_bytes(m))
        if nbytes <= 0:
            return False
        work = torch.empty(nbytes, dtype=torch.uint8, device=device)
        cb = _lib.BlockedPairs(m, T, P, 0, slabs[0].data_ptr(), slabs[1].data_ptr(), slabs[2].data_ptr(), words[0].data_ptr(),
                               words[1].data_ptr(), rows.data_ptr(), tok.data_ptr(), desc.data_ptr())
        st = C.c_void_p(torch.cuda.current_stream(device).cuda_stream)
        rc = lib.cfmm_blocked_build(m, hp.n_tokens, idx.data_ptr(), R.data_ptr(), gam.data_ptr(), C.byref(cb), order.data_ptr(),
                                    status.data_ptr(), work.data_ptr(), nbytes, st)
        if rc == -3:
            return False
        _lib.check(rc, "cfmm_blocked_build")
        st_h = status.cpu()
        if int(st_h[1]) != 0:
            raise ValueError("invalid pool data (reserves > 0 and finite, fees in (0, 1], two distinct token ids in range)")
        if int(st_h[0]) != 0:
            return False
        self.order = order
        self.residual = np.zeros(0, np.int64)
        self.m = m
        self.stride = M
        self.r0, self.r1, self.gamma_inv = slabs[0], slabs[1], slabs[2]
        self._keep = (idx, R, gam, work)
        self.tables = dict(n_tiles=T, M=M, lid=words[0], pos=words[1], rows=rows, tok=tok, desc=desc,
                           rows_per_pool=int(st_h[2]) / m, tok_per_tile=None)
        self.c_blocked = cb
        return True

    @property
    def sel(self) -> np.ndarray:
        if self._sel is None:
            self._sel = self.spec.sel[self.order.cpu().numpy().astype(np.int64)]
        return self._sel

    @property
    def off(self) -> np.ndarray:
        if self._off is None:
            self._off = self.spec.hp.pool_ptr[self.sel][None, :] + np.arange(2)[:, None]
        return self._off

    def bytes_resident(self) -> int:
        if self.tables is None:
            return 0
        ts = [self.r0, self.r1, self.gamma_inv] + [self.tables[k] for k in ("lid", "tok", "pos", "rows", "desc")]
        return sum(x.numel() * x.element_size() for x in ts)

    def out_struct(self, trades: bool, hess: bool):
        f64 = dict(dtype=torch.float64, device=self._device)
        if trades and self.delta is None:
            self.delta = torch.zeros((2, self.stride), **f64)
            self.lam = torch.zeros((2, self.stride), **f64)
        if hess and self.hcoef is None:
            self.hcoef = torch.zeros(self.stride, **f64)
        return _lib.EvalOut(self.delta.data_ptr() if trades else None, self.lam.data_ptr() if trades else None,
                            self.hcoef.data_ptr() if hess else None, None)


class PeerContext:

    def __init__(self, n_tokens: int, device, group):
        import torch.distributed as dist
        import torch.distributed._symmetric_memory as symm
        n = int(n_tokens)
        if n + 1 > 64 * 256:
            raise _lib.CfmmError("peer all-reduce supports n_tokens < 16384; use NCCL (Comm) beyond that")
        f64 = dict(dtype=torch.float64, device=device)
        self.group = group
        self.rank, self.world = dist.get_rank(group), dist.get_world_size(group)
        self.n_tokens = n
        w = self.world
        self.sym_acc = symm.empty((3 * w * (n + 1) * 2,), **f64); self.sym_acc.zero_()
        self.sym_y = symm.empty((3 * w * (n + 2) * 2,), **f64); self.sym_y.zero_()
        self.hdl_acc = symm.rendezvous(self.sym_acc, group)
        self.hdl_y = symm.rendezvous(self.sym_y, group)
        self.red_acc = torch.zeros(n + 1, **f64)
        self.red_y = torch.zeros(n, **f64)
        self.seq = [0, 0]
        torch.cuda.synchronize(device)
        dist.barrier(group)

    def next_seq(self, chan: int) -> int:
        self.seq[chan] += 1
        return self.seq[chan]

    def c_struct(self):
        return _lib.PeerCtx(int(self.hdl_acc.buffer_ptrs_dev), int(self.hdl_y.buffer_ptrs_dev), self.rank, self.world,
                            self.seq[0], self.seq[1])

    def absorb(self, c):
        self.seq = [int(c.seq_acc), int(c.seq_vec)]


_PEER_CONTEXTS: Dict[tuple, "PeerContext"] = {}


def peer_context(n_tokens: int, device, group=None) -> "PeerContext":
    import torch.distributed as dist
    group = group or dist.group.WORLD
    key = (int(n_tokens), id(group), str(torch.device(device)))
    if key not in _PEER_CONTEXTS:
        _PEER_CONTEXTS[key] = PeerContext(n_tokens, torch.device(device), group)
    return _PEER_CONTEXTS[key]


class PoolStore:

    def __init__(self, hp: HostPools, device="cuda", rank: int = 0, world: int = 1, validate: bool = True,
                 layout: str = "blocked"):
        if layout not in ("blocked", "plain"):
            raise ValueError("layout must be 'blocked' or 'plain'")
        if validate:
            if getattr(hp, "_uniform_product", False) and layout == "blocked":
                hp._validate_on_device = True
            else:
                hp.validate()
        self.lib = _lib.load()
        self.device = torch.device(device)
        if self.device.type != "cuda":
            raise _lib.CfmmError("PoolStore needs a CUDA device: there is no CPU path in this package")
        if not torch.cuda.is_available():
            raise _lib.CfmmError("no CUDA device visible: the routing kernels have no CPU fallback")
        self.n_tokens = int(hp.n_tokens)
        self.m_total = hp.m
        self.pool_ptr = hp.pool_ptr
        self._tok_idx_host = hp.tok_idx
        self.rank, self.world = rank, world
        self.buckets = []
        for s in split_buckets(hp, rank, world):
            if s.kind == _lib.KIND_PRODUCT and layout == "blocked" and s.m > 0:
                bb = BlockedBucket(hp, s, self.device, self.lib)
                if bb.m > 0:
                    self.buckets.append(bb)
                if len(bb.residual):
                    self.buckets.append(DeviceBucket(hp, s.subset(bb.residual), self.device))
            else:
                self.buckets.append(DeviceBucket(hp, s, self.device))
        self.buckets.sort(key=lambda b: 0 if getattr(b, "blocked", False) else 1)
        self._blocked_first = bool(self.buckets) and getattr(self.buckets[0], "blocked", False)
        assert sum(1 for b in self.buckets if getattr(b, "blocked", False)) <= 1
        self.m_local = sum(b.m for b in self.buckets)
        self.has_sum = bool(np.any(hp.kind == KIND_SUM_HOST))
        self.has_geomean = any(b.kind == _lib.KIND_GEOMEAN for b in self.buckets)
        f64 = dict(dtype=torch.float64, device=self.device)
        self._acc2 = torch.zeros((2, self.n_tokens + 1), **f64)
        self._y2 = torch.zeros((2, self.n_tokens), **f64)
        self._acc_i = 0
        self._y_i = 0
        self._move = torch.zeros(1, **f64)
        self.evals = 0
        self.hvps = 0

    def enable_peer_allreduce(self, group=None):
        self._peer = peer_context(self.n_tokens, self.device, group)
        self.reduces_internally = True

    def _peer_reduce(self, chan, local, n, st):
        p = self._peer
        seq = p.next_seq(chan)
        hdl, out = (p.hdl_acc, p.red_acc) if chan == 0 else (p.hdl_y, p.red_y)
        _lib.check(self.lib.cfmm_allreduce_ll(local.data_ptr(), int(hdl.buffer_ptrs_dev), p.rank, p.world, n,
                                              (seq % 3) * p.world * n, n, out.data_ptr(), seq, st), "cfmm_allreduce_ll")
        return out

    def _stream(self):
        return C.c_void_p(torch.cuda.current_stream(self.device).cuda_stream)

    def bytes_resident(self) -> int:
        return sum(b.bytes_resident() for b in self.buckets)

    def algorithmic_bytes_per_eval(self) -> int:
        n = 0
        for b in self.buckets:
            n += b.m * (28 * b.arity + 12 if b.kind == _lib.KIND_GEOMEAN else 48 if b.kind == _lib.KIND_BOUNDED else 32)
        return n + 16 * self.n_tokens + 8

    def evaluate(self, nu: torch.Tensor, eps: float = 0.0, trades: bool = False, hess: bool = False, reduce: bool = True):
        st = self._stream()
        acc = self._acc2[self._acc_i]
        nxt = self._acc2[self._acc_i ^ 1]
        self._acc_i ^= 1
        if not self._blocked_first:
            _lib.check(self.lib.cfmm_zero(acc.data_ptr(), acc.numel() * 8, st), "cfmm_zero")
        lognu = torch.log(nu) if self.has_geomean else None
        for b in self.buckets:
            out = b.out_struct(trades, hess) if (trades or hess) else None
            if getattr(b, "blocked", False):
                rc = self.lib.cfmm_blocked_eval(C.byref(b.c_blocked), self.n_tokens, nu.data_ptr(), acc.data_ptr(),
                                                acc.data_ptr() + 8 * self.n_tokens,
                                                C.byref(out) if out is not None else None,
                                                nxt.data_ptr(), nxt.numel(), st)
                _lib.check(rc, "cfmm_blocked_eval")
                continue
            rc = self.lib.cfmm_arb_eval(C.byref(b.c_bucket), self.n_tokens, nu.data_ptr(),
                                        lognu.data_ptr() if lognu is not None else None, float(eps),
                                        acc.data_ptr(), acc.data_ptr() + 8 * self.n_tokens,
                                        C.byref(out) if out is not None else None, st)
            _lib.check(rc, "cfmm_arb_eval")
        self.evals += 1
        if reduce and getattr(self, "reduces_internally", False):
            return self._peer_reduce(0, acc, self.n_tokens + 1, st)
        return acc

    def hvp(self, vt: torch.Tensor) -> torch.Tensor:
        st = self._stream()
        y = self._y2[self._y_i]
        ynxt = self._y2[self._y_i ^ 1]
        self._y_i ^= 1
        if not self._blocked_first:
            _lib.check(self.lib.cfmm_zero(y.data_ptr(), y.numel() * 8, st), "cfmm_zero")
        for b in self.buckets:
            if getattr(b, "blocked", False):
                _lib.check(self.lib.cfmm_blocked_hvp(C.byref(b.c_blocked), self.n_tokens, b.hcoef.data_ptr(),
                                                     vt.data_ptr(), y.data_ptr(), ynxt.data_ptr(), st),
                           "cfmm_blocked_hvp")
                continue
            rc = self.lib.cfmm_hvp(C.byref(b.c_bucket), self.n_tokens, b.hcoef.data_ptr(),
                                   b.hmask.data_ptr(), vt.data_ptr(), y.data_ptr(), st)
            _lib.check(rc, "cfmm_hvp")
        self.hvps += 1
        if getattr(self, "reduces_internally", False):
            return self._peer_reduce(1, y, self.n_tokens, st)
        return y

    def hess_diag(self) -> torch.Tensor:
        st = self._stream()
        d = torch.zeros(self.n_tokens, dtype=torch.float64, device=self.device)
        for b in self.buckets:
            if getattr(b, "blocked", False):
                _lib.check(self.lib.cfmm_blocked_diag(C.byref(b.c_blocked), self.n_tokens, b.hcoef.data_ptr(),
                                                      d.data_ptr(), st), "cfmm_blocked_diag")
                continue
            _lib.check(self.lib.cfmm_hess_diag(C.byref(b.c_bucket), self.n_tokens, b.hcoef.data_ptr(),
                                               b.hmask.data_ptr(), d.data_ptr(), st), "cfmm_hess_diag")
        if getattr(self, "reduces_internally", False):
            return self._peer_reduce(1, d, self.n_tokens, st).clone()
        return d

    def hess_dense(self) -> torch.Tensor:
        st = self._stream()
        H = torch.zeros((self.n_tokens, self.n_tokens), dtype=torch.float64, device=self.device)
        for b in self.buckets:
            if getattr(b, "blocked", False):
                _lib.check(self.lib.cfmm_blocked_dense(C.byref(b.c_blocked), self.n_tokens, b.hcoef.data_ptr(), H.data_ptr(), st),
                           "cfmm_blocked_dense")
                continue
            _lib.check(self.lib.cfmm_hess_dense(C.byref(b.c_bucket), self.n_tokens, b.hcoef.data_ptr(),
                                                b.hmask.data_ptr(), H.data_ptr(), st), "cfmm_hess_dense")
        return H

    def update_multipliers(self) -> torch.Tensor:
        st = self._stream()
        self._move.zero_()
        for b in self.buckets:
            if b.kind == _lib.KIND_SUM:
                _lib.check(self.lib.cfmm_sum_update_multipliers(C.byref(b.c_bucket), b.lam.data_ptr(),
                                                                b.theta_bar.data_ptr(), self._move.data_ptr(), st),
                           "cfmm_sum_update_multipliers")
        return self._move

    def reset_multipliers(self):
        for b in self.buckets:
            if b.theta_bar is not None:
                b.theta_bar.zero_()

    def gather_trades(self):
        nnz = int(self.pool_ptr[-1])
        delta = np.zeros(nnz); lam = np.zeros(nnz)
        for b in self.buckets:
            if b.m == 0:
                continue
            delta[b.off.ravel()] = b.delta[:, :b.m].cpu().numpy().ravel()
            lam[b.off.ravel()] = b.lam[:, :b.m].cpu().numpy().ravel()
        return delta, lam
```

### include/cfmm_b200.h

```cpp
#ifndef CFMM_B200_H
#define CFMM_B200_H

#include <stdint.h>

#ifdef __cplusplus
extern "C" {
#endif

enum {
    CFMM_KIND_PRODUCT = 0,
    CFMM_KIND_SUM = 1,
    CFMM_KIND_GEOMEAN = 2,
    CFMM_KIND_BOUNDED_PRODUCT = 3
};

enum {
    CFMM_OK = 0,
    CFMM_E_NULL = -1,
    CFMM_E_KIND = -2,
    CFMM_E_SIZE = -3,
    CFMM_E_CUDA = -4,
    CFMM_E_NODEVICE = -5,
    CFMM_E_STATE = -6
};

typedef struct cfmm_bucket {
    int32_t kind;
    int32_t arity;
    int64_t n_pools;
    int64_t stride;
    const double* reserves;
    const int32_t* tok_idx;
    const double* gamma;
    const double* weights;
    const double* logrw;
    const double* theta_bar;
} cfmm_bucket;

typedef struct cfmm_eval_out {
    double* delta;
    double* lambda;
    double* hcoef;
    uint32_t* hmask;
} cfmm_eval_out;

int cfmm_arb_eval(const cfmm_bucket* bucket, int32_t n_tokens, const double* nu, const double* log_nu,
                  double eps, double* psi, double* arb, const cfmm_eval_out* out, void* stream);

int cfmm_hvp(const cfmm_bucket* bucket, int32_t n_tokens, const double* hcoef, const uint32_t* hmask,
             const double* vt, double* y, void* stream);

int cfmm_hess_diag(const cfmm_bucket* bucket, int32_t n_tokens, const double* hcoef, const uint32_t* hmask,
                   double* diag, void* stream);

int cfmm_hess_dense(const cfmm_bucket* bucket, int32_t n_tokens, const double* hcoef, const uint32_t* hmask,
                    double* H, void* stream);

typedef struct cfmm_blocked_pairs {
    int64_t n_pools;
    int64_t n_tiles;
    int32_t pools_per_tile;
    int32_t reserved;
    const double* r0;
    const double* r1;
    const double* gamma_inv;
    const uint32_t* lid;
    const uint32_t* pos;
    const uint32_t* rows;
    const int32_t* tok;
    const int32_t* desc;
} cfmm_blocked_pairs;

int cfmm_blocked_layout_info(int32_t* pools_per_tile, int32_t* rows_stride, int32_t* tok_stride, int32_t* row_cap);
int cfmm_set_blocked_config(int32_t cfg);

int64_t cfmm_blocked_build_work_bytes(int64_t n_pools);
int cfmm_blocked_build(int64_t n_pools, int32_t n_tokens, const int32_t* idx, const double* reserves, const double* gamma,
                       const cfmm_blocked_pairs* out, uint32_t* order, int32_t* status, void* work, int64_t work_bytes,
                       void* stream);

int cfmm_blocked_eval(const cfmm_blocked_pairs* b, int32_t n_tokens, const double* nu, double* psi, double* arb,
                      const cfmm_eval_out* out, double* zero_next, int64_t n_zero, void* stream);
int cfmm_blocked_hvp(const cfmm_blocked_pairs* b, int32_t n_tokens, const double* hcoef, const double* vt, double* y,
                     double* zero_next, void* stream);
int cfmm_blocked_diag(const cfmm_blocked_pairs* b, int32_t n_tokens, const double* hcoef, double* diag, void* stream);
int cfmm_blocked_dense(const cfmm_blocked_pairs* b, int32_t n_tokens, const double* hcoef, double* H, void* stream);

typedef struct cfmm_solve_params {
    double tol;
    double nu_floor;
    int32_t max_iter;
    int32_t cg_max;
} cfmm_solve_params;

typedef struct cfmm_solve_result {
    double dual_value, primal_value, gap, primal_infeas, err;
    int32_t iters, evals, hvps, status;
} cfmm_solve_result;

int64_t cfmm_blocked_solve_work_bytes(const cfmm_blocked_pairs* b, int32_t n_tokens);
int cfmm_blocked_solve(const cfmm_blocked_pairs* b, int32_t n_tokens, const double* c, const double* a,
                       const uint8_t* eq, const uint8_t* pinned, double* nu, double* psi_out, void* work,
                       const cfmm_solve_params* prm, cfmm_solve_result* res, void* stream);

typedef struct cfmm_peer_ctx {
    const void* recv_acc_dev;
    const void* recv_vec_dev;
    int32_t rank, world;
    uint64_t seq_acc, seq_vec;
} cfmm_peer_ctx;

int cfmm_blocked_solve_peer(const cfmm_blocked_pairs* b, int32_t n_tokens, const double* c, const double* a,
                            const uint8_t* eq, const uint8_t* pinned, double* nu, double* psi_out, void* work,
                            const cfmm_solve_params* prm, cfmm_solve_result* res, cfmm_peer_ctx* peer, void* stream);

int64_t cfmm_persist_solve_work_bytes(const cfmm_blocked_pairs* b, int32_t n_tokens);
int cfmm_set_persist_cooperative(int32_t on);
int cfmm_persist_last_profile(int64_t* out8);
int cfmm_persist_solve(const cfmm_blocked_pairs* b, int32_t n_tokens, const double* c, const double* a,
                       const uint8_t* eq, const uint8_t* pinned, double* nu, double* psi_out, void* work,
                       const cfmm_solve_params* prm, cfmm_solve_result* res, cfmm_peer_ctx* peer, void* stream);

typedef struct cfmm_csr_pools {
    int32_t n_tokens;
    int64_t n_pools, nnz;
    const int64_t* pool_ptr;
    const int32_t* tok_idx;
    const double* reserves;
    const double* weights;
    const double* logrw;
    const double* gamma;
    const uint8_t* kind;
} cfmm_csr_pools;

typedef struct cfmm_batch {
    int32_t n_problems;
    const int64_t* pool_range;
    const double* c;
    const double* a;
    const uint8_t* flags;
    double* nu;
    double* psi;
    double* stats;
    double* delta;
    double* lambda;
    int64_t trade_stride;
} cfmm_batch;

typedef struct cfmm_batch_params {
    double tol;
    double eps0, eps_min, eps_shrink;
    double floor_rel;
    int32_t max_outer, max_inner;
} cfmm_batch_params;

int64_t cfmm_batch_solve_work_bytes(const cfmm_csr_pools* pools, int32_t n_problems, int64_t nnz_max);
int cfmm_set_batch_lanes(int32_t lanes);
int cfmm_batch_solve(const cfmm_csr_pools* pools, const cfmm_batch* batch, const cfmm_batch_params* prm, void* work,
                     void* stream);

int cfmm_allreduce_ll(const double* local, const void* peer_recv_dev, int32_t rank, int32_t world, int32_t n,
                      int64_t slot_off_cells, int64_t src_stride_cells, double* out, uint64_t seq, void* stream);

int cfmm_sum_update_multipliers(const cfmm_bucket* bucket, const double* lambda, double* theta_bar_out,
                                double* move, void* stream);

int cfmm_zero(void* ptr, int64_t bytes, void* stream);

int cfmm_set_scatter_mode(int32_t mode);

int64_t cfmm_launch_count(void);
void cfmm_reset_launch_count(void);
const char* cfmm_last_cuda_error(void);
const char* cfmm_version(void);

#ifdef __cplusplus
}
#endif
#endif
```

Before: 56.80 billion.

## Compress per-pool fee inverse into uint8 index into shared fee table

During layout build, the distinct gamma values are collected into a hash table. When there are at most 255 of them, each pool stores a one-byte fee index instead of an 8-byte gamma_inv, and the evaluation kernel looks the value up in a 256-entry table held in shared memory. This cuts the per-pool bytes streamed by TMA in the dual-evaluation pass, which is bandwidth-bound. It adds a build-time hash and rank step, extra kernel template variants, and a fallback to the full slab when there are too many distinct fees.

```diff
diff --git a/cfmm_routing_code_b200/_lib.py b/cfmm_routing_code_b200/_lib.py
--- a/cfmm_routing_code_b200/_lib.py
+++ b/cfmm_routing_code_b200/_lib.py
@@ -34,6 +34,7 @@
         ("n_pools", C.c_int64), ("n_tiles", C.c_int64), ("pools_per_tile", C.c_int32), ("reserved", C.c_int32),
         ("r0", C.c_void_p), ("r1", C.c_void_p), ("gamma_inv", C.c_void_p), ("lid", C.c_void_p),
         ("pos", C.c_void_p), ("rows", C.c_void_p), ("tok", C.c_void_p), ("desc", C.c_void_p),
+        ("fee_idx", C.c_void_p), ("fee_inv", C.c_void_p),
     ]
 
 
diff --git a/cfmm_routing_code_b200/csrc/cfmm_blocked.cu b/cfmm_routing_code_b200/csrc/cfmm_blocked.cu
--- a/cfmm_routing_code_b200/csrc/cfmm_blocked.cu
+++ b/cfmm_routing_code_b200/csrc/cfmm_blocked.cu
@@ -6,7 +6,7 @@
 
 namespace {
 
-template <int P, int THREADS, int STAGES, int MODE , bool TRADES, bool HESS>
+template <int P, int THREADS, int STAGES, int MODE , bool TRADES, bool HESS, bool FIDX>
 __global__ void __launch_bounds__(THREADS, kCtasPerSm)
 k_blocked(const BlockedArgs A) {
     extern __shared__ __align__(128) unsigned char smem_raw[];
@@ -21,7 +21,7 @@
     const long long t_end = (A.n_tiles * (long long)(blockIdx.x + 1)) / gridDim.x;
     double acc = 0.0, acc2 = 0.0;
     unsigned phase = 0;
-    blocked_pass<P, THREADS, STAGES, MODE, TRADES, HESS, false, true>(A, smem_raw, full, phase, t_beg, t_end, acc, acc2);
+    blocked_pass<P, THREADS, STAGES, MODE, TRADES, HESS, false, true, FIDX>(A, smem_raw, full, phase, t_beg, t_end, acc, acc2);
     if (MODE == 0) cta_accumulate<THREADS>(acc, part, A.arb);
 }
 
@@ -228,11 +228,11 @@
 int g_pdl = 1;
 int g_row_cap = 32;
 
-template <int MODE, bool TRADES, bool HESS>
-int launch_tma(const BlockedArgs& A, cudaStream_t st) {
+template <int MODE, bool TRADES, bool HESS, bool FIDX>
+int launch_tma_v(const BlockedArgs& A, cudaStream_t st) {
     constexpr int NF = (MODE == 0) ? 3 : 1;
-    auto kern = k_blocked<kTileP, kTileT, kTileStages, MODE, TRADES, HESS>;
-    const size_t sm = pass_smem_bytes<kTileP, kTileStages>(NF);
+    auto kern = k_blocked<kTileP, kTileT, kTileStages, MODE, TRADES, HESS, FIDX>;
+    const size_t sm = pass_smem_bytes<kTileP, kTileStages>(NF, FIDX);
     static bool attr = false;
     if (!attr) {
         cudaFuncSetAttribute(kern, cudaFuncAttributeMaxDynamicSharedMemorySize, (int)sm);
@@ -248,6 +248,11 @@
     cfg.attrs = at; cfg.numAttrs = 1;
     cudaLaunchKernelEx(&cfg, kern, A);
     return check_launch();
+}
+
+template <int MODE, bool TRADES, bool HESS>
+int launch_tma(const BlockedArgs& A, cudaStream_t st) {
+    return A.fee_idx ? launch_tma_v<MODE, TRADES, HESS, true>(A, st) : launch_tma_v<MODE, TRADES, HESS, false>(A, st);
 }
 
 template <int MODE>
@@ -287,8 +292,20 @@
     A.desc = reinterpret_cast<const int4*>(b->desc);
     A.zero_next = nullptr; A.n_zero = 0;
     A.slab[0] = A.slab[1] = A.slab[2] = nullptr;
+    A.fee_idx = nullptr; A.fee_inv = nullptr;
     A.vec = nullptr; A.vec2 = nullptr; A.beta = 0.0;
     A.out = nullptr; A.arb = nullptr; A.delta = A.lambda = A.hcoef = nullptr;
+    return CFMM_OK;
+}
+
+int fill_blocked_slabs(const cfmm_blocked_pairs* b, BlockedArgs& A) {
+    if (!b->r0 || !b->r1 || !b->gamma_inv) return CFMM_E_NULL;
+    A.slab[0] = b->r0; A.slab[1] = b->r1; A.slab[2] = b->gamma_inv;
+    if (b->fee_idx) {
+        if (!b->fee_inv) return CFMM_E_NULL;
+        if (reinterpret_cast<uintptr_t>(b->fee_idx) & 15u) return CFMM_E_SIZE;
+        A.fee_idx = b->fee_idx; A.fee_inv = b->fee_inv;
+    }
     return CFMM_OK;
 }
 
@@ -318,8 +335,8 @@
     if (n_tokens <= 0) return CFMM_E_SIZE;
     if (!nu || !psi || !arb) return CFMM_E_NULL;
     if (b->n_tiles == 0) return CFMM_OK;
-    if (!b->r0 || !b->r1 || !b->gamma_inv) return CFMM_E_NULL;
-    A.slab[0] = b->r0; A.slab[1] = b->r1; A.slab[2] = b->gamma_inv;
+    rc = fill_blocked_slabs(b, A);
+    if (rc) return rc;
     A.vec = nu; A.out = psi; A.arb = arb;
     A.zero_next = zero_next; A.n_zero = zero_next ? (int)n_zero : 0;
     const bool trades = out && out->delta && out->lambda;
diff --git a/cfmm_routing_code_b200/csrc/cfmm_blocked.cuh b/cfmm_routing_code_b200/csrc/cfmm_blocked.cuh
--- a/cfmm_routing_code_b200/csrc/cfmm_blocked.cuh
+++ b/cfmm_routing_code_b200/csrc/cfmm_blocked.cuh
@@ -15,6 +15,7 @@
 constexpr int kTileT = kTileP / 2;
 constexpr int kTileStages = 2;
 constexpr int kCtasPerSm = CFMM_CTAS_PER_SM;
+constexpr int kFeeTable = 256;
 static_assert(kTileP % 64 == 0 && kTileP <= 1024, "tile size: whole warps of two-pool threads, 10-bit local token ids");
 
 template <int P>
@@ -24,8 +25,15 @@
     static constexpr int kRowsMax = P + 2 * P / kRowCapMin + 8;
 };
 
-template <int P, int NF>
-struct __align__(128) Stage {
+template <int P, bool FIDX>
+struct StageFee {};
+template <int P>
+struct StageFee<P, true> {
+    uint8_t fid[P];
+};
+
+template <int P, int NF, bool FIDX = false>
+struct __align__(128) Stage : StageFee<P, FIDX> {
     double a[NF][P];
     uint32_t lid[P];
     uint32_t pos[P];
@@ -38,6 +46,8 @@
     long long n_tiles;
     long long M;
     const double* slab[3];
+    const uint8_t* fee_idx;
+    const double* fee_inv;
     const uint32_t* lid;
     const uint32_t* pos;
     const uint32_t* rows;
@@ -57,16 +67,17 @@
 
 __device__ __forceinline__ unsigned round16(unsigned bytes) { return (bytes + 15u) & ~15u; }
 
-template <int P, int NF>
-__device__ __forceinline__ void issue_tile(Stage<P, NF>* st, uint64_t* bar, const BlockedArgs& A, long long tile,
+template <int P, int NF, bool FIDX>
+__device__ __forceinline__ void issue_tile(Stage<P, NF, FIDX>* st, uint64_t* bar, const BlockedArgs& A, long long tile,
                                            const int4 d) {
     const unsigned rows_b = round16(4u * (unsigned)d.y);
     const unsigned tok_b = round16(4u * (unsigned)d.x);
     const long long off = tile * P;
-    mbar_expect_tx(bar, (unsigned)(NF * P * 8 + P * 4 + P * 4 + 16) + rows_b + tok_b);
+    mbar_expect_tx(bar, (unsigned)(NF * P * 8 + (FIDX ? P : 0) + P * 4 + P * 4 + 16) + rows_b + tok_b);
     bulk_g2s(&st->desc, A.desc + tile, 16, bar);
 #pragma unroll
     for (int k = 0; k < NF; ++k) bulk_g2s(st->a[k], A.slab[k] + off, P * 8, bar);
+    if constexpr (FIDX) bulk_g2s(st->fid, A.fee_idx + off, P, bar);
     bulk_g2s(st->lid, A.lid + off, P * 4, bar);
     bulk_g2s(st->pos, A.pos + off, P * 4, bar);
     bulk_g2s(st->rows, A.rows + tile * BlockedCfg<P>::kRowsMax, rows_b, bar);
@@ -115,24 +126,31 @@
 }
 
 template <int P, int STAGES>
-constexpr size_t pass_smem_bytes(int nf) {
-    return (size_t)STAGES * (nf == 3 ? sizeof(Stage<P, 3>) : sizeof(Stage<P, 1>)) + (size_t)(3 * P) * sizeof(double);
-}
-
-template <int P, int THREADS, int STAGES, int MODE, bool TRADES, bool HESS, bool COHERENT, bool PDL>
+constexpr size_t pass_smem_bytes(int nf, bool fidx = false) {
+    return nf == 1 ? (size_t)STAGES * sizeof(Stage<P, 1>) + (size_t)(3 * P) * sizeof(double)
+           : fidx  ? (size_t)STAGES * sizeof(Stage<P, 2, true>) + (size_t)(3 * P + kFeeTable) * sizeof(double)
+                   : (size_t)STAGES * sizeof(Stage<P, 3>) + (size_t)(3 * P) * sizeof(double);
+}
+
+template <int P, int THREADS, int STAGES, int MODE, bool TRADES, bool HESS, bool COHERENT, bool PDL, bool FIDX = false>
 __device__ __forceinline__ void blocked_pass(const BlockedArgs& A, unsigned char* smem_raw, uint64_t* full, unsigned& phase,
                                              long long t_beg, long long t_end, double& acc, double& acc2) {
-    constexpr int NF = (MODE == 0) ? 3 : 1;
-    using St = Stage<P, NF>;
+    static_assert(!FIDX || MODE == 0, "only the evaluation reads gamma");
+    constexpr int NF = (MODE == 0) ? (FIDX ? 2 : 3) : 1;
+    using St = Stage<P, NF, FIDX>;
     St* stages = reinterpret_cast<St*>(smem_raw);
     double* nul = reinterpret_cast<double*>(smem_raw + (size_t)STAGES * sizeof(St));
     double* g = nul + P;
+    double* finv = g + 2 * P;
     const int tid = threadIdx.x;
     if (tid == 0) {
         for (int s = 0; s < STAGES; ++s) {
             const long long t = t_beg + s;
-            if (t < t_end) issue_tile<P, NF>(&stages[s], &full[s], A, t, __ldg(A.desc + t));
-        }
+            if (t < t_end) issue_tile<P, NF, FIDX>(&stages[s], &full[s], A, t, __ldg(A.desc + t));
+        }
+    }
+    if (FIDX) {
+        for (int k = tid; k < kFeeTable; k += THREADS) finv[k] = __ldg(A.fee_inv + k);
     }
     if (PDL) {
         asm volatile("griddepcontrol.wait;" ::: "memory");
@@ -166,7 +184,10 @@
                 const uint32_t li = S.lid[l];
                 ps[u] = S.pos[l];
                 if (MODE == 0) {
-                    EvalOp::apply<TRADES, HESS>(A, tile * P + l, S.a[0][l], S.a[NF > 1 ? 1 : 0][l], S.a[NF > 2 ? 2 : 0][l],
+                    double gi;
+                    if constexpr (FIDX) gi = finv[S.fid[l]];
+                    else gi = S.a[NF > 2 ? 2 : 0][l];
+                    EvalOp::apply<TRADES, HESS>(A, tile * P + l, S.a[0][l], S.a[NF > 1 ? 1 : 0][l], gi,
                                                 nul[li & 0xffffu], nul[li >> 16], f0[u], f1[u], acc);
                 } else if (MODE == 1) {
                     const double pa = nul[li & 0xffffu], pb = nul[li >> 16], h = S.a[0][l];
@@ -226,7 +247,7 @@
         __syncthreads();
         if (tid == 0 && far < t_end) {
             fence_proxy_async();
-            issue_tile<P, NF>(&S, &full[stage], A, far, dfar);
+            issue_tile<P, NF, FIDX>(&S, &full[stage], A, far, dfar);
         }
         stage = nstage;
     }
@@ -246,5 +267,6 @@
 }
 
 int fill_blocked_args(const cfmm_blocked_pairs* b, BlockedArgs& A);
-
-}
+int fill_blocked_slabs(const cfmm_blocked_pairs* b, BlockedArgs& A);
+
+}
diff --git a/cfmm_routing_code_b200/csrc/cfmm_layout.cu b/cfmm_routing_code_b200/csrc/cfmm_layout.cu
--- a/cfmm_routing_code_b200/csrc/cfmm_layout.cu
+++ b/cfmm_routing_code_b200/csrc/cfmm_layout.cu
@@ -21,6 +21,9 @@
     const double* gamma;
     const uint32_t* order;
     double *r0, *r1, *gi;
+    uint8_t* fid;
+    const unsigned long long* fee_keys;
+    const int32_t* fee_rank;
     uint32_t *lid, *pos;
     uint32_t* rows;
     int32_t* tok;
@@ -28,9 +31,35 @@
     int32_t* status;
 };
 
+constexpr int kFeeHash = 512;
+constexpr int kFeeMax = kFeeTable - 1;
+
+__device__ __forceinline__ unsigned fee_slot(unsigned long long bits) {
+    return (unsigned)((bits * 0x9E3779B97F4A7C15ull) >> 55);
+}
+__device__ __forceinline__ int fee_insert(unsigned long long* tab, unsigned long long bits) {
+    unsigned s = fee_slot(bits);
+    for (int k = 0; k < kFeeHash; ++k, s = (s + 1) & (kFeeHash - 1)) {
+        unsigned long long cur = *reinterpret_cast<volatile unsigned long long*>(tab + s);
+        if (cur == 0ull) cur = atomicCAS(tab + s, 0ull, bits);
+        if (cur == 0ull) return 1;
+        if (cur == bits) return 0;
+    }
+    return -1;
+}
+
 __global__ void __launch_bounds__(256)
 k_pool_keys(long long m, int n_tokens, int nb, const int32_t* __restrict__ idx, const double* __restrict__ R,
-            const double* __restrict__ gamma, uint32_t* __restrict__ keys, uint32_t* __restrict__ vals, int32_t* status) {
+            const double* __restrict__ gamma, uint32_t* __restrict__ keys, uint32_t* __restrict__ vals, int32_t* status,
+            unsigned long long* fee_keys, int* fee_count) {
+    __shared__ unsigned long long fee_s[kFeeHash];
+    __shared__ int fee_n;
+    const bool fees = fee_keys != nullptr;
+    if (fees) {
+        for (int k = threadIdx.x; k < kFeeHash; k += blockDim.x) fee_s[k] = 0ull;
+        if (threadIdx.x == 0) fee_n = 0;
+        __syncthreads();
+    }
     int bad = 0;
     for (long long i = (long long)blockIdx.x * blockDim.x + threadIdx.x; i < m; i += (long long)gridDim.x * blockDim.x) {
         const int a = idx[2 * i], b = idx[2 * i + 1];
@@ -41,8 +70,50 @@
         const long long ba = ok ? ((long long)a * nb) / n_tokens : 0, bb = ok ? ((long long)b * nb) / n_tokens : 0;
         keys[i] = (uint32_t)((ba * nb + bb) * n_tokens + (ok ? a : 0));
         vals[i] = (uint32_t)i;
+        if (fees && ok && *reinterpret_cast<volatile int*>(&fee_n) <= kFeeMax &&
+            fee_insert(fee_s, (unsigned long long)__double_as_longlong(g)) > 0)
+            atomicAdd(&fee_n, 1);
     }
     if (__syncthreads_or(bad) && threadIdx.x == 0) atomicAdd(status + 1, 1);
+    if (!fees) return;
+    if (fee_n > kFeeMax) {
+        if (threadIdx.x == 0) status[3] = 1;
+        return;
+    }
+    for (int k = threadIdx.x; k < kFeeHash; k += blockDim.x) {
+        const unsigned long long bits = fee_s[k];
+        if (bits == 0ull || *reinterpret_cast<volatile int32_t*>(status + 3)) continue;
+        const int r = fee_insert(fee_keys, bits);
+        if (r < 0 || (r > 0 && atomicAdd(fee_count, 1) >= kFeeMax)) status[3] = 1;
+    }
+}
+
+__global__ void __launch_bounds__(kFeeHash)
+k_fee_table(const unsigned long long* __restrict__ fee_keys, int32_t* __restrict__ fee_rank, double* __restrict__ fee_inv) {
+    __shared__ unsigned long long ks[kFeeHash];
+    const int t = threadIdx.x;
+    const unsigned long long mine = fee_keys[t];
+    ks[t] = mine;
+    const int n = __syncthreads_count(mine != 0ull);
+    int rank = 0;
+    for (int k = 0; k < kFeeHash; ++k) {
+        const unsigned long long o = ks[k];
+        rank += (o != 0ull && o < mine) ? 1 : 0;
+    }
+    fee_rank[t] = mine != 0ull ? rank : kFeeMax;
+    if (mine != 0ull && rank < kFeeMax) fee_inv[rank] = 1.0 / __longlong_as_double((long long)mine);
+    if (t < kFeeTable && t >= (n < kFeeMax ? n : kFeeMax)) fee_inv[t] = 1.0;
+}
+
+__device__ __forceinline__ uint8_t fee_index(const BuildArgs& B, double g) {
+    const unsigned long long bits = (unsigned long long)__double_as_longlong(g);
+    unsigned s = fee_slot(bits);
+    for (int k = 0; k < kFeeHash; ++k, s = (s + 1) & (kFeeHash - 1)) {
+        const unsigned long long cur = B.fee_keys[s];
+        if (cur == bits) return (uint8_t)min(B.fee_rank[s], kFeeMax);
+        if (cur == 0ull) break;
+    }
+    return (uint8_t)kFeeMax;
 }
 
 using Sort = cub::BlockRadixSort<uint32_t, LT, LI, uint32_t>;
@@ -118,6 +189,7 @@
         if (tid == 0) { atomicAdd(B.status, 1); B.desc[tile] = make_int4(0, 0, 0, 0); }
         for (int l = tid; l < LP; l += LT) {
             B.r0[p0 + l] = 1.0; B.r1[p0 + l] = 1.0; B.gi[p0 + l] = 1.0; B.lid[p0 + l] = 0u; B.pos[p0 + l] = 0u;
+            if (B.fid) B.fid[p0 + l] = (uint8_t)kFeeMax;
         }
         return;
     }
@@ -187,18 +259,23 @@
             B.lid[p0 + l] = (uint32_t)lidh[l][0] | (uint32_t)lidh[l][1] << 16;
             B.pos[p0 + l] = (uint32_t)posh[l][0] | (uint32_t)posh[l][1] << 16;
             B.r0[p0 + l] = B.R[2 * (long long)pool]; B.r1[p0 + l] = B.R[2 * (long long)pool + 1];
-            B.gi[p0 + l] = 1.0 / B.gamma[pool];
+            const double g = B.gamma[pool];
+            B.gi[p0 + l] = 1.0 / g;
+            if (B.fid) B.fid[p0 + l] = fee_index(B, g);
         } else {
             const int pl = l - np;
             B.lid[p0 + l] = 0u;
             B.pos[p0 + l] = (uint32_t)(nh + 2 * pl) | (uint32_t)(nh + 2 * pl + 1) << 16;
             B.r0[p0 + l] = 1.0; B.r1[p0 + l] = 1.0; B.gi[p0 + l] = 1.0;
+            if (B.fid) B.fid[p0 + l] = (uint8_t)kFeeMax;
         }
     }
     if (tid == 0) { B.desc[tile] = make_int4(s_ntok, s_nrow, 0, 0); atomicAdd(B.status + 2, s_nrow); }
 }
 
 inline size_t align_up(size_t x) { return (x + 255) & ~(size_t)255; }
+
+constexpr size_t kFeeWorkBytes = 8 * kFeeHash + 4 * kFeeHash + 16;
 
 size_t sort_temp_bytes(long long m) {
     size_t bytes = 0;
@@ -213,7 +290,7 @@
 
 int64_t cfmm_blocked_build_work_bytes(int64_t n_pools) {
     if (n_pools <= 0 || n_pools > 0x7fffffffLL) return CFMM_E_SIZE;
-    return (int64_t)(4 * align_up(4 * (size_t)n_pools) + align_up(sort_temp_bytes(n_pools)));
+    return (int64_t)(4 * align_up(4 * (size_t)n_pools) + align_up(sort_temp_bytes(n_pools)) + align_up(kFeeWorkBytes));
 }
 
 int cfmm_blocked_build(int64_t n_pools, int32_t n_tokens, const int32_t* idx, const double* reserves, const double* gamma,
@@ -241,19 +318,33 @@
     take(4 * (size_t)n_pools);
     size_t temp_bytes = sort_temp_bytes(n_pools);
     void* temp = take(temp_bytes);
+    unsigned char* fee_work = take(kFeeWorkBytes);
+    unsigned long long* fee_keys = reinterpret_cast<unsigned long long*>(fee_work);
+    int32_t* fee_rank = reinterpret_cast<int32_t*>(fee_work + 8 * kFeeHash);
+    int* fee_count = reinterpret_cast<int*>(fee_work + 12 * kFeeHash);
+    const bool fees = out->fee_idx && out->fee_inv;
     cudaMemsetAsync(status, 0, 16, st);
+    if (fees) cudaMemsetAsync(fee_work, 0, kFeeWorkBytes, st);
     const int grid = (int)((n_pools + 255) / 256 < 4LL * num_sms() ? (n_pools + 255) / 256 : 4LL * num_sms());
-    k_pool_keys<<<grid, 256, 0, st>>>(n_pools, n_tokens, (int)nb, idx, reserves, gamma, keys, vals, status);
+    k_pool_keys<<<grid, 256, 0, st>>>(n_pools, n_tokens, (int)nb, idx, reserves, gamma, keys, vals, status,
+                                      fees ? fee_keys : nullptr, fee_count);
     int rc = check_launch();
     if (rc) return rc;
     if (cub::DeviceRadixSort::SortPairs(temp, temp_bytes, keys, keys2, vals, order, (int)n_pools, 0, key_bits, st) != cudaSuccess) {
         g_last_err = cudaGetLastError();
         return CFMM_E_CUDA;
     }
+    if (fees) {
+        k_fee_table<<<1, kFeeHash, 0, st>>>(fee_keys, fee_rank, const_cast<double*>(out->fee_inv));
+        rc = check_launch();
+        if (rc) return rc;
+    }
     BuildArgs B;
     B.m = n_pools; B.n_tokens = n_tokens; B.nb = (int)nb; B.row_cap = row_cap; B.key_bits = key_bits; B.tok_bits = 32;
     B.idx = idx; B.R = reserves; B.gamma = gamma; B.order = order;
     B.r0 = const_cast<double*>(out->r0); B.r1 = const_cast<double*>(out->r1); B.gi = const_cast<double*>(out->gamma_inv);
+    B.fid = fees ? const_cast<uint8_t*>(out->fee_idx) : nullptr;
+    B.fee_keys = fee_keys; B.fee_rank = fee_rank;
     B.lid = const_cast<uint32_t*>(out->lid); B.pos = const_cast<uint32_t*>(out->pos);
     B.rows = const_cast<uint32_t*>(out->rows); B.tok = const_cast<int32_t*>(out->tok);
     B.desc = reinterpret_cast<int4*>(const_cast<int32_t*>(out->desc));
diff --git a/cfmm_routing_code_b200/csrc/cfmm_persist.cu b/cfmm_routing_code_b200/csrc/cfmm_persist.cu
--- a/cfmm_routing_code_b200/csrc/cfmm_persist.cu
+++ b/cfmm_routing_code_b200/csrc/cfmm_persist.cu
@@ -47,7 +47,7 @@
 
 struct Kkt { double err, g, primal, infeas, lin; };
 
-template <int MODE>
+template <int MODE, bool FIDX>
 __device__ __forceinline__ void run_pass(const PersistArgs& S, const double* vec, double* out, unsigned char* smem_raw,
                                          uint64_t* full, unsigned& phase, long long t_beg, long long t_end, double* part,
                                          double beta) {
@@ -58,7 +58,8 @@
     else A.slab[0] = S.hcoef;
     if (MODE == 1) { A.vec2 = S.z; A.beta = beta; }
     double acc = 0.0, acc2 = 0.0;
-    blocked_pass<kTileP, PT, kTileStages, MODE, false, MODE == 0, true, false>(A, smem_raw, full, phase, t_beg, t_end, acc, acc2);
+    blocked_pass<kTileP, PT, kTileStages, MODE, false, MODE == 0, true, false, FIDX && MODE == 0>(A, smem_raw, full, phase,
+                                                                                                    t_beg, t_end, acc, acc2);
     if (MODE == 0) {
         cta_accumulate<PT>(acc, part, A.arb);
         asm volatile("fence.proxy.async;" ::: "memory");
@@ -147,7 +148,7 @@
     return s;
 }
 
-template <bool MULTI>
+template <bool MULTI, bool FIDX>
 __global__ void __launch_bounds__(PT, kCtasPerSm)
 k_solve_dist(const __grid_constant__ DistArgs D) {
     extern __shared__ __align__(128) unsigned char smem_raw[];
@@ -188,9 +189,9 @@
         const int phase = ds.phase, set = ds.set, cur = ds.cur;
         if (phase == PH_DONE || ds.aborted) break;
         const long long tp0 = clock64();
-        if (phase == PH_KKT) run_pass<0>(S, S.nu[set], S.acc[set], smem_raw, full, phase_bits, t_beg, t_end, part, 0.0);
-        else if (phase == PH_HVP) run_pass<1>(S, S.p, D.y2[ds.yb], smem_raw, full, phase_bits, t_beg, t_end, part, ds.beta);
-        else if (phase == PH_DIAG) run_pass<2>(S, nullptr, S.diag, smem_raw, full, phase_bits, t_beg, t_end, part, 0.0);
+        if (phase == PH_KKT) run_pass<0, FIDX>(S, S.nu[set], S.acc[set], smem_raw, full, phase_bits, t_beg, t_end, part, 0.0);
+        else if (phase == PH_HVP) run_pass<1, FIDX>(S, S.p, D.y2[ds.yb], smem_raw, full, phase_bits, t_beg, t_end, part, ds.beta);
+        else if (phase == PH_DIAG) run_pass<2, FIDX>(S, nullptr, S.diag, smem_raw, full, phase_bits, t_beg, t_end, part, 0.0);
         const long long tp1 = clock64();
         if (phase != PH_STEP) grid_barrier(S.ctl, &ds);
         const long long tp2 = clock64();
@@ -441,7 +442,6 @@
                        const cfmm_solve_params* prm, cfmm_solve_result* res, cfmm_peer_ctx* peer, void* stream) {
     if (!b || !c || !a || !eq || !pinned || !nu || !psi_out || !work || !prm || !res) return CFMM_E_NULL;
     if (n_tokens <= 0 || b->n_tiles <= 0) return CFMM_E_SIZE;
-    if (!b->r0 || !b->r1 || !b->gamma_inv) return CFMM_E_NULL;
     if (peer && (!peer->recv_acc_dev || !peer->recv_vec_dev)) return CFMM_E_NULL;
     if (peer && (peer->world < 2 || peer->world > 16 || peer->rank < 0 || peer->rank >= peer->world)) return CFMM_E_SIZE;
     cudaStream_t st = static_cast<cudaStream_t>(stream);
@@ -449,7 +449,8 @@
     memset(&S, 0, sizeof(S));
     int rc = fill_blocked_args(b, S.B);
     if (rc) return rc;
-    S.B.slab[0] = b->r0; S.B.slab[1] = b->r1; S.B.slab[2] = b->gamma_inv;
+    rc = fill_blocked_slabs(b, S.B);
+    if (rc) return rc;
     const int n = n_tokens;
     S.n = n; S.c = c; S.a = a; S.eq = eq; S.fixed = pinned;
     unsigned char* w = static_cast<unsigned char*>(work);
@@ -480,11 +481,12 @@
     D.partial = reinterpret_cast<double*>(take(8 * (size_t)2 * kQ * kSliceMax));
     D.nsl = (n + 15) / 16 < kSliceMax ? ((n + 15) / 16 > 0 ? (n + 15) / 16 : 1) : kSliceMax;
     D.P = S;
-    const size_t sm = pass_smem_bytes<kTileP, kTileStages>(3);
-    const bool multi = S.world > 1;
-    auto kern = multi ? k_solve_dist<true> : k_solve_dist<false>;
-    static int occs[2] = {-1, -1};
-    int& occ = occs[multi ? 1 : 0];
+    const bool multi = S.world > 1, fidx = S.B.fee_idx != nullptr;
+    const size_t sm = pass_smem_bytes<kTileP, kTileStages>(3, fidx);
+    auto kern = multi ? (fidx ? k_solve_dist<true, true> : k_solve_dist<true, false>)
+                      : (fidx ? k_solve_dist<false, true> : k_solve_dist<false, false>);
+    static int occs[4] = {-1, -1, -1, -1};
+    int& occ = occs[(multi ? 2 : 0) + (fidx ? 1 : 0)];
     if (occ < 0) {
         int o = -1;
         cudaError_t e = cudaFuncSetAttribute(kern, cudaFuncAttributeMaxDynamicSharedMemorySize, (int)sm);
diff --git a/cfmm_routing_code_b200/pools.py b/cfmm_routing_code_b200/pools.py
--- a/cfmm_routing_code_b200/pools.py
+++ b/cfmm_routing_code_b200/pools.py
@@ -335,6 +335,20 @@
     return order, residual, tables
 
 
+FEE_TABLE = 256
+
+
+def fee_table(gamma: torch.Tensor, M: int):
+    uniq, inv = torch.unique(gamma, sorted=True, return_inverse=True)
+    if uniq.numel() > FEE_TABLE - 1:
+        return None, None
+    fee_idx = torch.full((M,), FEE_TABLE - 1, dtype=torch.uint8, device=gamma.device)
+    fee_idx[:gamma.numel()] = inv.to(torch.uint8)
+    fee_inv = torch.ones(FEE_TABLE, dtype=torch.float64, device=gamma.device)
+    fee_inv[:uniq.numel()] = 1.0 / uniq
+    return fee_idx, fee_inv
+
+
 class BlockedBucket:
     kind = _lib.KIND_PRODUCT
     arity = 2
@@ -346,6 +360,7 @@
         f64 = dict(dtype=torch.float64, device=device)
         self.theta_bar = None
         self.delta = self.lam = self.hcoef = self.hmask = None
+        self.fee_idx = self.fee_inv = None
         self._device = device
         self._sel = self._off = None
         if spec.identity and int(hp.pool_ptr[-1]) == 2 * hp.m and self._build_native(hp, spec, device, lib, P, rows_stride, tok_stride):
@@ -381,10 +396,13 @@
             return out
         self.r0 = slab(R[order, 0], 1.0)
         self.r1 = slab(R[order, 1], 1.0)
-        self.gamma_inv = slab(1.0 / gam[order], 1.0)
+        g = gam[order]
+        self.gamma_inv = slab(1.0 / g, 1.0)
+        self.fee_idx, self.fee_inv = fee_table(g, t["M"])
         self.c_blocked = _lib.BlockedPairs(self.m, t["n_tiles"], P, 0, self.r0.data_ptr(), self.r1.data_ptr(),
                                            self.gamma_inv.data_ptr(), t["lid"].data_ptr(), t["pos"].data_ptr(),
-                                           t["rows"].data_ptr(), t["tok"].data_ptr(), t["desc"].data_ptr())
+                                           t["rows"].data_ptr(), t["tok"].data_ptr(), t["desc"].data_ptr(),
+                                           *self._fee_ptrs())
 
     def _build_native(self, hp, spec, device, lib, P, rows_stride, tok_stride) -> bool:
         lo, hi = spec.lo, spec.hi
@@ -408,12 +426,15 @@
         desc = torch.empty((T, 4), **i32)
         order = torch.empty(m, **i32)
         status = torch.empty(4, **i32)
+        fee_idx = torch.empty(M, dtype=torch.uint8, device=device)
+        fee_inv = torch.empty(FEE_TABLE, **f64)
         nbytes = int(lib.cfmm_blocked_build_work_bytes(m))
         if nbytes <= 0:
             return False
         work = torch.empty(nbytes, dtype=torch.uint8, device=device)
         cb = _lib.BlockedPairs(m, T, P, 0, slabs[0].data_ptr(), slabs[1].data_ptr(), slabs[2].data_ptr(), words[0].data_ptr(),
-                               words[1].data_ptr(), rows.data_ptr(), tok.data_ptr(), desc.data_ptr())
+                               words[1].data_ptr(), rows.data_ptr(), tok.data_ptr(), desc.data_ptr(), fee_idx.data_ptr(),
+                               fee_inv.data_ptr())
         st = C.c_void_p(torch.cuda.current_stream(device).cuda_stream)
         rc = lib.cfmm_blocked_build(m, hp.n_tokens, idx.data_ptr(), R.data_ptr(), gam.data_ptr(), C.byref(cb), order.data_ptr(),
                                     status.data_ptr(), work.data_ptr(), nbytes, st)
@@ -430,6 +451,10 @@
         self.m = m
         self.stride = M
         self.r0, self.r1, self.gamma_inv = slabs[0], slabs[1], slabs[2]
+        if int(st_h[3]) != 0:
+            fee_idx = fee_inv = None
+            cb.fee_idx = cb.fee_inv = None
+        self.fee_idx, self.fee_inv = fee_idx, fee_inv
         self._keep = (idx, R, gam, work)
         self.tables = dict(n_tiles=T, M=M, lid=words[0], pos=words[1], rows=rows, tok=tok, desc=desc,
                            rows_per_pool=int(st_h[2]) / m, tok_per_tile=None)
@@ -448,10 +473,16 @@
             self._off = self.spec.hp.pool_ptr[self.sel][None, :] + np.arange(2)[:, None]
         return self._off
 
+    def _fee_ptrs(self):
+        if self.fee_idx is None:
+            return None, None
+        return self.fee_idx.data_ptr(), self.fee_inv.data_ptr()
+
     def bytes_resident(self) -> int:
         if self.tables is None:
             return 0
         ts = [self.r0, self.r1, self.gamma_inv] + [self.tables[k] for k in ("lid", "tok", "pos", "rows", "desc")]
+        ts += [x for x in (self.fee_idx, self.fee_inv) if x is not None]
         return sum(x.numel() * x.element_size() for x in ts)
 
     def out_struct(self, trades: bool, hess: bool):
diff --git a/include/cfmm_b200.h b/include/cfmm_b200.h
--- a/include/cfmm_b200.h
+++ b/include/cfmm_b200.h
@@ -69,6 +69,8 @@
     const uint32_t* rows;
     const int32_t* tok;
     const int32_t* desc;
+    const uint8_t* fee_idx;
+    const double* fee_inv;
 } cfmm_blocked_pairs;
 
 int cfmm_blocked_layout_info(int32_t* pools_per_tile, int32_t* rows_stride, int32_t* tok_stride, int32_t* row_cap);
```

After: 59.55 billion, median of 6. 4.8% higher.
